# lmjakt/kmer_hasheR

Hardware: NVIDIA B200
Metric: kmers_indexed_per_s (higher is better)
Workload: dtype u64

## Files before the change

### kmer_hasher_b200/csrc/api.cu

```cuda
#include <cstdarg>
#include <cstdio>
#include <cstring>
#include <ctime>
#include <algorithm>
#include <atomic>
#include <condition_variable>
#include <deque>
#include <thread>
#include <map>
#include <mutex>
#include <string>
#include <type_traits>
#include <vector>

#include "../../include/kmergpu.h"
#include "common.cuh"
#include "csr.cuh"
#include "lookback.cuh"
#include "probe.cuh"
#include "sort.cuh"
#include "windows.cuh"

using namespace kmg;

static thread_local char g_err[512] = "";
static int fail(int code, const char *fmt, ...) {
  va_list ap;
  va_start(ap, fmt);
  vsnprintf(g_err, sizeof g_err, fmt, ap);
  va_end(ap);
  return code;
}
#define CU(call)                                                                                   \
  do {                                                                                             \
    cudaError_t e_ = (call);                                                                       \
    if (e_ != cudaSuccess) {                                                                       \
      int code_ = (e_ == cudaErrorMemoryAllocation) ? KMG_ERR_NOMEM                                \
                  : (e_ == cudaErrorNoDevice || e_ == cudaErrorInsufficientDriver) ? KMG_ERR_NODEV \
                                                                                   : KMG_ERR_CUDA; \
      return fail(code_, "%s: %s (%s:%d)", #call, cudaGetErrorString(e_), __FILE__, __LINE__);     \
    }                                                                                              \
  } while (0)
#define TRY(call)            \
  do {                       \
    int rc_ = (call);        \
    if (rc_ != KMG_OK) return rc_; \
  } while (0)

extern "C" const char *kmg_last_error(void) { return g_err; }
extern "C" int kmg_version(void) { return 100; }

struct Ctx {
  int device = 0;
  bool ready = false;
  cudaStream_t own = nullptr, copy = nullptr;
  cudaStream_t user = nullptr;
  bool use_user = false;
  cudaEvent_t ev[8] = {nullptr, nullptr, nullptr, nullptr, nullptr, nullptr, nullptr, nullptr};
  int sms = 148;
  cudaStream_t stream() const { return use_user ? user : own; }
};
static thread_local Ctx g_ctx;

static int ctx_init() {
  Ctx &c = g_ctx;
  if (c.ready) {
    CU(cudaSetDevice(c.device));
    return KMG_OK;
  }
  int n = 0;
  cudaError_t e = cudaGetDeviceCount(&n);
  if (e != cudaSuccess || n == 0)
    return fail(KMG_ERR_NODEV, "no CUDA device: %s (libkmergpu has no CPU path)", cudaGetErrorString(e));
  if (c.device >= n) return fail(KMG_ERR_ARG, "device %d out of range (have %d)", c.device, n);
  CU(cudaSetDevice(c.device));
  cudaDeviceProp prop;
  CU(cudaGetDeviceProperties(&prop, c.device));
  if (prop.major != 10 || prop.minor != 0)
    return fail(KMG_ERR_NODEV, "device %d is sm_%d%d; libkmergpu is built for sm_100a (B200) only", c.device, prop.major, prop.minor);
  c.sms = prop.multiProcessorCount;
  CU(cudaStreamCreateWithFlags(&c.own, cudaStreamNonBlocking));
  CU(cudaStreamCreateWithFlags(&c.copy, cudaStreamNonBlocking));
  for (auto &ev : c.ev) CU(cudaEventCreateWithFlags(&ev, cudaEventDisableTiming));
  c.ready = true;
  return KMG_OK;
}

extern "C" int kmg_device_count(int *n) {
  if (!n) return fail(KMG_ERR_ARG, "n is NULL");
  cudaError_t e = cudaGetDeviceCount(n);
  if (e != cudaSuccess) { *n = 0; return fail(KMG_ERR_NODEV, "cudaGetDeviceCount: %s", cudaGetErrorString(e)); }
  return KMG_OK;
}
extern "C" int kmg_set_device(int device) {
  if (device < 0) return fail(KMG_ERR_ARG, "negative device");
  if (g_ctx.ready && g_ctx.device != device) {
    g_ctx = Ctx();
  }
  g_ctx.device = device;
  return ctx_init();
}
extern "C" int kmg_set_stream(void *s) {
  g_ctx.user = (cudaStream_t)s;
  g_ctx.use_user = true;
  return KMG_OK;
}
extern "C" int kmg_unset_stream(void) { g_ctx.use_user = false; return KMG_OK; }
extern "C" void *kmg_host_alloc(size_t bytes) {
  void *p = nullptr;
  if (ctx_init() != KMG_OK) return nullptr;
  if (cudaMallocHost(&p, bytes ? bytes : 1) != cudaSuccess) { fail(KMG_ERR_NOMEM, "cudaMallocHost(%zu) failed", bytes); return nullptr; }
  return p;
}
extern "C" void kmg_host_free(void *p) { if (p) cudaFreeHost(p); }

struct ProfEntry { double ms = 0; uint64_t launches = 0; double bytes = 0; };
struct ProfPending { std::string name; cudaEvent_t a, b; };
static std::mutex g_prof_mu;
static bool g_prof_on = false;
static std::map<std::string, ProfEntry> g_prof;
static std::vector<ProfPending> g_prof_pending;
static std::vector<cudaEvent_t> g_prof_free;
static uint64_t g_launches = 0;

static cudaEvent_t prof_event() {
  if (!g_prof_free.empty()) { cudaEvent_t e = g_prof_free.back(); g_prof_free.pop_back(); return e; }
  cudaEvent_t e;
  cudaEventCreate(&e);
  return e;
}
static void prof_resolve() {
  for (auto &p : g_prof_pending) {
    float ms = 0;
    if (cudaEventSynchronize(p.b) == cudaSuccess && cudaEventElapsedTime(&ms, p.a, p.b) == cudaSuccess) {
      g_prof[p.name].ms += ms;
    }
    g_prof_free.push_back(p.a);
    g_prof_free.push_back(p.b);
  }
  g_prof_pending.clear();
}
struct LaunchScope {
  const char *name;
  cudaStream_t s;
  cudaEvent_t a = nullptr, b = nullptr;
  bool on;
  LaunchScope(const char *n, cudaStream_t st) : name(n), s(st) {
    std::lock_guard<std::mutex> g(g_prof_mu);
    on = g_prof_on;
    ++g_launches;
    if (on) { a = prof_event(); b = prof_event(); cudaEventRecord(a, s); }
  }
  ~LaunchScope() {
    if (!on) return;
    cudaEventRecord(b, s);
    std::lock_guard<std::mutex> g(g_prof_mu);
    g_prof[name].launches++;
    g_prof_pending.push_back({name, a, b});
  }
};
static void prof_bytes(const char *name, double bytes) {
  std::lock_guard<std::mutex> g(g_prof_mu);
  if (g_prof_on) g_prof[name].bytes += bytes;
}
#define LAUNCH(name, stream, ...)                                                              \
  do {                                                                                         \
    { LaunchScope ls_(name, stream); __VA_ARGS__; }                                            \
    cudaError_t le_ = cudaGetLastError();                                                      \
    if (le_ != cudaSuccess) return fail(KMG_ERR_CUDA, "launch %s: %s", name, cudaGetErrorString(le_)); \
  } while (0)

extern "C" int kmg_profile_enable(int on) { std::lock_guard<std::mutex> g(g_prof_mu); g_prof_on = on != 0; return KMG_OK; }
extern "C" int kmg_profile_reset(void) {
  std::lock_guard<std::mutex> g(g_prof_mu);
  prof_resolve();
  g_prof.clear();
  return KMG_OK;
}
extern "C" int kmg_profile_count(void) {
  std::lock_guard<std::mutex> g(g_prof_mu);
  prof_resolve();
  return (int)g_prof.size();
}
extern "C" int kmg_profile_get(int i, const char **name, double *total_ms, uint64_t *launches, double *algo_bytes) {
  std::lock_guard<std::mutex> g(g_prof_mu);
  prof_resolve();
  if (i < 0 || i >= (int)g_prof.size()) return fail(KMG_ERR_ARG, "profile index out of range");
  auto it = g_prof.begin();
  std::advance(it, i);
  if (name) *name = it->first.c_str();
  if (total_ms) *total_ms = it->second.ms;
  if (launches) *launches = it->second.launches;
  if (algo_bytes) *algo_bytes = it->second.bytes;
  return KMG_OK;
}
extern "C" uint64_t kmg_launch_count(void) { std::lock_guard<std::mutex> g(g_prof_mu); return g_launches; }

struct Arena {
  struct Block { void *p; size_t cap; cudaStream_t last; bool synced; };
  std::mutex mu;
  std::multimap<size_t, Block> cache;
  std::map<void *, Block> live;
  size_t cached_bytes = 0, limit = 0;

  static size_t round_up(size_t bytes) {
    if (bytes < (size_t(1) << 20)) return (bytes + 511) & ~size_t(511);
    return (bytes + (size_t(2) << 20) - 1) & ~((size_t(2) << 20) - 1);
  }
  void trim_locked() {
    for (auto &kv : cache) cudaFree(kv.second.p);
    cache.clear();
    cached_bytes = 0;
  }
  int get(void **out, size_t bytes, cudaStream_t s) {
    const size_t cap = round_up(bytes ? bytes : 1);
    std::unique_lock<std::mutex> g(mu);
    auto it = cache.lower_bound(cap);
    if (it != cache.end() && it->first <= cap + std::max(cap / 4, size_t(1) << 20)) {
      Block b = it->second;
      cache.erase(it);
      cached_bytes -= b.cap;
      g.unlock();
      if (!b.synced && b.last != s) cudaStreamSynchronize(b.last);
      g.lock();
      b.last = s; b.synced = false;
      live[b.p] = b;
      *out = b.p;
      return KMG_OK;
    }
    void *p = nullptr;
    cudaError_t e = cudaMalloc(&p, cap);
    if (e != cudaSuccess) {
      cudaGetLastError();
      trim_locked();
      e = cudaMalloc(&p, cap);
    }
    if (e != cudaSuccess) { cudaGetLastError(); return fail(KMG_ERR_NOMEM, "device allocation of %zu bytes failed: %s", cap, cudaGetErrorString(e)); }
    live[p] = Block{p, cap, s, false};
    *out = p;
    return KMG_OK;
  }
  void put(void *p, cudaStream_t s, bool synced) {
    if (!p) return;
    std::lock_guard<std::mutex> g(mu);
    auto it = live.find(p);
    if (it == live.end()) {
      for (auto &kv : cache) if (kv.second.p == p) return;
      cudaFree(p);
      return;
    }
    Block b = it->second;
    live.erase(it);
    b.last = s; b.synced = synced;
    if (limit == 0) {
      const char *e = getenv("KMERGPU_CACHE_MB");
      size_t fr = 0, tot = 0;
      if (e && atoll(e) >= 0) limit = (size_t)atoll(e) << 20;
      else limit = cudaMemGetInfo(&fr, &tot) == cudaSuccess ? tot / 4 : (size_t(32) << 30);
      if (limit == 0) limit = 1;
    }
    if (cached_bytes + b.cap > limit) trim_locked();
    cache.emplace(b.cap, b);
    cached_bytes += b.cap;
  }
};
static Arena g_arena[64];

static void stage_release();
extern "C" int kmg_trim(void) {
  TRY(ctx_init());
  cudaStreamSynchronize(g_ctx.stream());
  Arena &a = g_arena[g_ctx.device & 63];
  std::lock_guard<std::mutex> g(a.mu);
  for (auto &kv : a.cache) if (!kv.second.synced && kv.second.last && kv.second.last != g_ctx.stream()) cudaStreamSynchronize(kv.second.last);
  a.trim_locked();
  stage_release();
  return KMG_OK;
}
extern "C" uint64_t kmg_cached_bytes(void) {
  Arena &a = g_arena[g_ctx.device & 63];
  std::lock_guard<std::mutex> g(a.mu);
  return a.cached_bytes;
}

template <typename T>
static int dalloc(T **p, size_t count, cudaStream_t s) {
  *p = nullptr;
  return g_arena[g_ctx.device & 63].get((void **)p, (count ? count : 1) * sizeof(T), s);
}
template <typename T>
static void dfree(T *&p, cudaStream_t s) {
  if (p) g_arena[g_ctx.device & 63].put((void *)p, s, false);
  p = nullptr;
}

extern "C" void kmg_host_copy(void *dst, const void *src, size_t n);
class CopyPool {
  struct Task { char *dst; const char *src; size_t n; int group; };
  std::mutex mu;
  std::condition_variable cv_work, cv_done;
  std::deque<Task> q;
  int pending[8] = {0, 0, 0, 0, 0, 0, 0, 0};
  std::vector<std::thread> th;
  bool stop = false;
  void run() {
    for (;;) {
      Task t;
      {
        std::unique_lock<std::mutex> l(mu);
        cv_work.wait(l, [&] { return stop || !q.empty(); });
        if (q.empty()) return;
        t = q.front();
        q.pop_front();
      }
      kmg_host_copy(t.dst, t.src, t.n);
      {
        std::lock_guard<std::mutex> l(mu);
        if (--pending[t.group & 7] == 0) cv_done.notify_all();
      }
    }
  }
 public:
  int threads() {
    std::lock_guard<std::mutex> l(mu);
    if (th.empty()) {
      const char *e = getenv("KMERGPU_COPY_THREADS");
      int n = e ? atoi(e) : (int)std::thread::hardware_concurrency() / 2;
      n = std::max(1, std::min(n, 8));
      for (int i = 0; i < n; ++i) th.emplace_back([this] { run(); });
    }
    return (int)th.size();
  }
  void submit(int group, void *dst, const void *src, size_t n) {
    const int parts = threads();
    const size_t piece = ((n + parts - 1) / parts + 4095) & ~size_t(4095);
    std::lock_guard<std::mutex> l(mu);
    for (size_t off = 0; off < n; off += piece) {
      q.push_back(Task{(char *)dst + off, (const char *)src + off, std::min(piece, n - off), group});
      ++pending[group & 7];
    }
    cv_work.notify_all();
  }
  void wait(int group) {
    std::unique_lock<std::mutex> l(mu);
    cv_done.wait(l, [&] { return pending[group & 7] == 0; });
  }
  ~CopyPool() {
    { std::lock_guard<std::mutex> l(mu); stop = true; }
    cv_work.notify_all();
    for (auto &t : th) t.join();
  }
};
static CopyPool g_pool;
constexpr size_t STAGE_BYTES = size_t(64) << 20;
constexpr int STAGE_SLOTS = 3;
struct Staging {
  std::mutex mu;
  char *slot[STAGE_SLOTS] = {nullptr, nullptr, nullptr};
  int ensure() {
    for (auto &p : slot)
      if (!p && cudaMallocHost((void **)&p, STAGE_BYTES) != cudaSuccess) { cudaGetLastError(); return fail(KMG_ERR_NOMEM, "pinned staging allocation failed"); }
    return KMG_OK;
  }
  void release() { for (auto &p : slot) { if (p) cudaFreeHost(p); p = nullptr; } }
};
static Staging g_stage;
static void stage_release() { std::lock_guard<std::mutex> gs(g_stage.mu); g_stage.release(); }
static bool staged_transfers() {
  static int on = -1;
  if (on < 0) { const char *e = getenv("KMERGPU_STAGING"); on = !(e && e[0] == '0'); }
  return on == 1;
}

static int staged_upload(void *d_dst, const void *h_src, size_t bytes, cudaStream_t s) {
  std::lock_guard<std::mutex> g(g_stage.mu);
  TRY(g_stage.ensure());
  cudaEvent_t *ev = g_ctx.ev + 4;
  int c = 0;
  for (size_t off = 0; off < bytes; off += STAGE_BYTES, ++c) {
    const int sl = c % STAGE_SLOTS;
    const size_t n = std::min(STAGE_BYTES, bytes - off);
    if (c >= STAGE_SLOTS) CU(cudaEventSynchronize(ev[sl]));
    g_pool.submit(c, g_stage.slot[sl], (const char *)h_src + off, n);
    g_pool.wait(c);
    CU(cudaMemcpyAsync((char *)d_dst + off, g_stage.slot[sl], n, cudaMemcpyHostToDevice, s));
    CU(cudaEventRecord(ev[sl], s));
  }
  CU(cudaStreamSynchronize(s));
  return KMG_OK;
}

enum PtrKind { PK_HOST_PAGEABLE, PK_HOST_PINNED, PK_DEVICE };
static PtrKind ptr_kind(const void *p) {
  cudaPointerAttributes a;
  if (cudaPointerGetAttributes(&a, p) != cudaSuccess) { cudaGetLastError(); return PK_HOST_PAGEABLE; }
  if (a.type == cudaMemoryTypeDevice || a.type == cudaMemoryTypeManaged) return PK_DEVICE;
  if (a.type == cudaMemoryTypeHost) return PK_HOST_PINNED;
  return PK_HOST_PAGEABLE;
}

struct DevSeq {
  uint8_t *buf = nullptr;
  uint8_t *base = nullptr;
  int64_t len = 0;
};
static int upload_seq(const void *src, int64_t len, cudaStream_t s, DevSeq *out) {
  size_t cap = 16 + (size_t)((len + 15) / 16) * 16 + 16;
  TRY(dalloc(&out->buf, cap, s));
  out->base = out->buf + 16;
  out->len = len;
  CU(cudaMemsetAsync(out->buf, 0, 16, s));
  CU(cudaMemsetAsync(out->buf + cap - 32, 0, 32, s));
  if (len > (int64_t)(8 << 20) && staged_transfers() && ptr_kind(src) == PK_HOST_PAGEABLE) return staged_upload(out->base, src, (size_t)len, s);
  if (len > 0) CU(cudaMemcpyAsync(out->base, src, (size_t)len, cudaMemcpyDefault, s));
  return KMG_OK;
}

struct kmg_index {
  int device = 0;
  int k = 0;
  uint64_t U = 0, N = 0;
  uint64_t P = 0, multi = 0;
  uint32_t maxc = 0;
  bool have_stats = false;
  bool grouped = false;
  int hbits = 0;
  bool unstable = false;
  uint64_t *ukeys = nullptr;
  uint32_t *ustart = nullptr;
  uint32_t *pos = nullptr;
  std::mutex mu;
  uint4 *hash = nullptr;
  uint64_t hash_nb = 0;
  int hash_hbits = 0;
  uint32_t *multi_u = nullptr;
  uint64_t *pair_off = nullptr;
};
struct kmg_query {
  const kmg_index *idx = nullptr;
  uint64_t H = 0, M = 0;
  int32_t *hit_i = nullptr;
  uint32_t *hit_start = nullptr;
  uint64_t *row_off = nullptr;
};

constexpr int HIST_THREADS = 512, HIST_ITEMS = 16, HIST_TILE = HIST_THREADS * HIST_ITEMS;
constexpr int RLE_THREADS = 256, RLE_ITEMS = 16, RLE_TILE = RLE_THREADS * RLE_ITEMS;
constexpr int PROBE_THREADS = 256, PROBE_ITEMS = 8, PROBE_TILE = PROBE_THREADS * PROBE_ITEMS;
constexpr int COMPACT_ITEMS = 8, COMPACT_TILE = PROBE_THREADS * COMPACT_ITEMS;
constexpr int EMIT_THREADS = 256, EMIT_TILE = EMIT_THREADS * 8;
constexpr int PIDX_THREADS = 256, PIDX_ITEMS = 8, PIDX_TILE = PIDX_THREADS * PIDX_ITEMS;

static int g_sort_shape = -1;
static int g_rank_override = -1;
static std::atomic<int> g_rank_dev[64];
static std::atomic<uint64_t> g_unstable_rebuilds{0};
static std::atomic<uint64_t> g_region_rebuilds{0};
static uint32_t g_sort_dbg = 0;
static int lane_order_failures(uint32_t *failures);
static bool log_on();

static int rank_variant() {
  if (g_rank_override >= 0) return g_rank_override;
  const int dev = g_ctx.device & 63;
  int v = g_rank_dev[dev].load(std::memory_order_acquire);
  if (v == 0) {
    const char *e = getenv("KMG_SORT_RANK");
    if (e) v = atoi(e) == 3 ? 2 : 1;
    else {
      uint32_t f = 1;
      v = (lane_order_failures(&f) == KMG_OK && f == 0) ? 2 : 1;
      if (log_on()) fprintf(stderr, "[kmergpu] device %d lane-order self-test: %u failures -> rank variant %d\n", dev, f, v == 2 ? 3 : 0);
    }
    int expect = 0;
    g_rank_dev[dev].compare_exchange_strong(expect, v, std::memory_order_acq_rel);
    v = g_rank_dev[dev].load(std::memory_order_acquire);
  }
  return v == 2 ? 3 : 0;
}
static void demote_rank_variant() {
  g_rank_dev[g_ctx.device & 63].store(1, std::memory_order_release);
  g_unstable_rebuilds.fetch_add(1);
  if (g_rank_override >= 3) g_rank_override = -1;
  if (log_on()) fprintf(stderr, "[kmergpu] device %d: position lists not ascending after a one-atomic sort pass; switching to the bitmap variant\n", g_ctx.device);
}

struct SortPlan { int rb, passes; int bits() const { return rb * passes; } };
static int g_hash_bits = 0;
static int g_hash_rb = 0;
static int g_no_regions = 0;
static int g_scatter_shape = 0;
static int g_scatter_bitmap = 0;
static int g_hash_cas = 0;
static int g_fix_cap = 0;
static SortPlan grouped_plan(int64_t n_upper) {
  if (g_hash_bits > 0) {
    const int rb = g_hash_rb > 0 && g_hash_bits % g_hash_rb == 0 ? g_hash_rb : (g_hash_bits % 8 == 0 ? 8 : 9);
    return SortPlan{rb, g_hash_bits / rb};
  }
  if (g_hash_rb > 0) return SortPlan{g_hash_rb, (36 + g_hash_rb - 1) / g_hash_rb};
  return n_upper <= (int64_t)400000000 ? SortPlan{8, 4} : SortPlan{8, 5};
}
static bool grouped_for(int k, int order, int64_t ) {
  return order == KMG_ORDER_GROUPED && 2 * k > 40;
}

static unsigned long long *g_trace = nullptr;
static int g_trace_tiles = 0;
extern "C" int kmg_trace_read(unsigned long long *host, int tiles) {
  if (!g_trace || tiles > g_trace_tiles) return -1;
  return cudaMemcpy(host, g_trace, (size_t)tiles * 64, cudaMemcpyDeviceToHost) == cudaSuccess ? 0 : -4;
}
extern "C" int kmg_tune(const char *key, int value) {
  if (key && !strcmp(key, "sort_cfg")) {
    if (value != -1 && value != 0 && value != 3 && value != 4) return fail(KMG_ERR_ARG, "sort_cfg must be -1 (auto), 0 (bitmap), 3 (one atomic) or 4 (tests: unstable on purpose)");
    g_rank_override = value;
    return KMG_OK;
  }
  if (key && !strcmp(key, "sort_shape")) {
    if (value < -1 || value > 2) return fail(KMG_ERR_ARG, "sort_shape out of range");
    g_sort_shape = value;
    return KMG_OK;
  }
  if (key && !strcmp(key, "sort_dbg")) { g_sort_dbg = (uint32_t)value; return KMG_OK; }
  if (key && !strcmp(key, "fix_cap")) { g_fix_cap = value > 0 ? value : 0; return KMG_OK; }
  if (key && !strcmp(key, "hash_cas")) { g_hash_cas = value != 0; return KMG_OK; }
  if (key && !strcmp(key, "scatter_bitmap")) { g_scatter_bitmap = value != 0; return KMG_OK; }
  if (key && !strcmp(key, "scatter_shape")) { g_scatter_shape = value; return KMG_OK; }
  if (key && !strcmp(key, "no_regions")) { g_no_regions = value; return KMG_OK; }
  if (key && !strcmp(key, "hash_bits")) {
    if (value != 0 && (value < 8 || value > 56 || (value % 8 && value % 9 && value % 10))) return fail(KMG_ERR_ARG, "hash_bits must be 0 (auto) or a multiple of 8, 9 or 10 in [8,56]");
    g_hash_bits = value;
    return KMG_OK;
  }
  if (key && !strcmp(key, "hash_rb")) {
    if (value != 0 && (value < 8 || value > 10)) return fail(KMG_ERR_ARG, "hash_rb must be 0, 8, 9 or 10");
    g_hash_rb = value;
    return KMG_OK;
  }
  if (key && !strcmp(key, "reset_rank")) {
    for (auto &v : g_rank_dev) v.store(0);
    return KMG_OK;
  }
  if (key && !strcmp(key, "sort_trace")) {
    if (g_trace) { cudaFree(g_trace); g_trace = nullptr; }
    g_trace_tiles = value;
    if (value > 0) { if (cudaMalloc(&g_trace, (size_t)value * 64) != cudaSuccess) return fail(KMG_ERR_NOMEM, "trace alloc"); cudaMemset(g_trace, 0, (size_t)value * 64); }
    return KMG_OK;
  }
  return fail(KMG_ERR_ARG, "unknown tuning key");
}
extern "C" int64_t kmg_tune_get(const char *key, int64_t arg) {
  if (key && !strcmp(key, "rank_variant")) return ctx_init() == KMG_OK ? rank_variant() : -1;
  if (key && !strcmp(key, "unstable_rebuilds")) return (int64_t)g_unstable_rebuilds.load();
  if (key && !strcmp(key, "region_rebuilds")) return (int64_t)g_region_rebuilds.load();
  if (key && !strcmp(key, "hash_bits")) return grouped_plan(arg).bits();
  if (key && !strcmp(key, "hash_rb")) return grouped_plan(arg).rb;
  return -1;
}
static int lane_order_failures(uint32_t *failures) {
  TRY(ctx_init());
  cudaStream_t s = g_ctx.stream();
  uint32_t *bad = nullptr;
  TRY(dalloc(&bad, 1, s));
  CU(cudaMemsetAsync(bad, 0, 4, s));
  LAUNCH("lane_order_selftest", s, lane_order_selftest_kernel<<<g_ctx.sms * 4, 256, 0, s>>>(bad));
  CU(cudaMemcpyAsync(failures, bad, 4, cudaMemcpyDeviceToHost, s));
  CU(cudaStreamSynchronize(s));
  dfree(bad, s);
  return KMG_OK;
}
extern "C" int kmg_selftest_lane_order(uint32_t *failures) {
  if (!failures) return fail(KMG_ERR_ARG, "failures is NULL");
  return lane_order_failures(failures);
}
static_assert(2 * (sizeof(PassSmem<PassCfg<256, 28, 2, 3, 4, 8>, false>) + 1024) <= 196 * 1024, "the record pass's tile outgrew the 196 KB carve-out");
constexpr int REGION_SAMPLE_STRIDE = 251;
constexpr int SORT_TILE_MIN = 4096;

template <class Cfg, bool FROM_SEQ, class BinFn, class NextFn, bool HAS_NEXT, bool PEER = false, bool SEGS = false>
static int launch_pass_cfg(const char *name, const PassParams<BinFn, NextFn> &P, int64_t n_upper, cudaStream_t s, int extra_tiles = 0) {
  using S = PassSmem<Cfg, FROM_SEQ>;
  if constexpr (!FROM_SEQ && !PEER && !SEGS) {
    if (P.segs) return launch_pass_cfg<Cfg, FROM_SEQ, BinFn, NextFn, HAS_NEXT, PEER, true>(name, P, n_upper, s, extra_tiles);
  }
  auto kern = scatter_pass_kernel<Cfg, FROM_SEQ, BinFn, NextFn, HAS_NEXT, PEER, SEGS>;
  CU(cudaFuncSetAttribute(kern, cudaFuncAttributeMaxDynamicSharedMemorySize, (int)sizeof(S)));
  const int64_t tiles = ceil_div<int64_t>(n_upper, Cfg::TILE) + extra_tiles;
  if (tiles == 0) return KMG_OK;
  LAUNCH(name, s, kern<<<(unsigned)tiles, Cfg::THREADS, sizeof(S), s>>>(P));
  return KMG_OK;
}
template <bool FROM_SEQ, class BinFn, class NextFn, bool HAS_NEXT>
static int launch_pass(const char *name, const PassParams<BinFn, NextFn> &P, int64_t n_upper, cudaStream_t s, int rb = RADIX_BITS, int extra_tiles = 0) {
  const int rank = rank_variant();
  const int shape = g_sort_shape < 0 ? (rb == 8 ? 1 : 0)
                                     : (rb == 8) ? ((FROM_SEQ && g_sort_shape == 0) ? 1 : g_sort_shape) : (g_sort_shape == 2 ? 0 : g_sort_shape);
#define KMG_GO(T, I, M, RK, RB) return launch_pass_cfg<PassCfg<T, I, M, RK, (RK >= 3 ? 4 : 8), RB>, FROM_SEQ, BinFn, NextFn, HAS_NEXT>(name, P, n_upper, s, extra_tiles)
#define KMG_SHAPES(RK, RB)                         \
  do {                                             \
    if (shape == 1) KMG_GO(256, 28, 2, RK, RB);    \
    KMG_GO(256, 24, 2, RK, RB);                    \
  } while (0)
  if (rb == 8) {
    if (rank == 4) KMG_GO(256, 24, 2, 4, 8);
    if (shape == 2) { if (rank == 3) KMG_GO(256, 20, 3, 3, 8); else KMG_GO(256, 20, 3, 0, 8); }
    if (rank == 3) KMG_SHAPES(3, 8); else KMG_SHAPES(0, 8);
  } else if (rb == 9) {
    if (rank == 4) KMG_GO(256, 24, 2, 4, 9);
    if (rank == 3) KMG_SHAPES(3, 9); else KMG_SHAPES(0, 9);
  } else if (rb == 10) {
    if (rank == 3) KMG_GO(256, 24, 2, 3, 10); else KMG_GO(256, 24, 2, 0, 10);
  }
#undef KMG_SHAPES
#undef KMG_GO
  return fail(KMG_ERR_ARG, "bad sort configuration");
}

static uint32_t record_tile(int rb) {
  const int shape = g_sort_shape < 0 ? (rb == 8 ? 1 : 0) : (rb == 8) ? g_sort_shape : (g_sort_shape == 2 ? 0 : g_sort_shape);
  if (rank_variant() == 4 || rb == 10) return 256 * 24;
  return shape == 1 ? 256 * 28 : shape == 2 ? 256 * 20 : 256 * 24;
}

struct SortScratch {
  uint32_t *small = nullptr;
  uint64_t *status = nullptr;
  size_t small_words = 0, status_words = 0;
  static constexpr size_t H = (size_t)(MAX_PASSES + 1) * MAX_NB;
  uint32_t *hist(int r) const { return small + (size_t)r * MAX_NB; }
  uint32_t *gbase(int r) const { return small + H + (size_t)r * MAX_NB; }
  uint32_t *common() const { return small + 2 * H; }
  uint32_t *ticket(int i) const { return small + 2 * H + RADIX + i; }
  IndexStats *stats() const { return reinterpret_cast<IndexStats *>(small + 2 * H + RADIX + 16); }
};
static int scratch_clear(SortScratch &sc, cudaStream_t s) {
  CU(cudaMemsetAsync(sc.small, 0, sc.small_words * 4, s));
  CU(cudaMemsetAsync(sc.status, 0, sc.status_words * sizeof(uint64_t), s));
  return KMG_OK;
}
static int scratch_alloc(SortScratch &sc, int64_t n_upper, cudaStream_t s, int rb = RADIX_BITS) {
  sc.small_words = 2 * SortScratch::H + RADIX + 16 + sizeof(IndexStats) / 4;
  TRY(dalloc(&sc.small, sc.small_words, s));
  const size_t tiles = (size_t)ceil_div<int64_t>(n_upper > 0 ? n_upper : 1, SORT_TILE_MIN) + MAX_SEGS + 1;
  sc.status_words = tiles << rb;
  TRY(dalloc(&sc.status, sc.status_words, s));
  return scratch_clear(sc, s);
}
static void scratch_free(SortScratch &sc, cudaStream_t s) { dfree(sc.small, s); dfree(sc.status, s); }

template <class... A>
static int launch_scan_hist(int rb, cudaStream_t s, A... args) {
  if (rb == 8) LAUNCH("scan_hist", s, scan_hist_kernel<256><<<1, 256, 0, s>>>(args...));
  else if (rb == 9) LAUNCH("scan_hist", s, scan_hist_kernel<512><<<1, 512, 0, s>>>(args...));
  else if (rb == 10) LAUNCH("scan_hist", s, scan_hist_kernel<1024><<<1, 1024, 0, s>>>(args...));
  else return fail(KMG_ERR_ARG, "bad digit width");
  return KMG_OK;
}

static int finish_index(kmg_index *ix, SortScratch &sc, uint64_t *keys_sorted, uint32_t *pos_sorted,
                        int64_t n_upper, cudaStream_t s, bool hashed = false) {
  IndexStats *st = sc.stats();
  uint64_t *ukeys = nullptr;
  uint32_t *ustart = nullptr;
  Pair64 *status2 = nullptr;
  const int64_t tiles = ceil_div<int64_t>(n_upper > 0 ? n_upper : 1, RLE_TILE);
  TRY(dalloc(&ukeys, (size_t)n_upper, s));
  TRY(dalloc(&ustart, (size_t)n_upper + 1, s));
  TRY(dalloc(&status2, (size_t)tiles, s));
  CU(cudaMemsetAsync(status2, 0, (size_t)tiles * sizeof(Pair64), s));
  LAUNCH("rle", s, rle_kernel<RLE_THREADS, RLE_ITEMS><<<(unsigned)tiles, RLE_THREADS, 0, s>>>(
                       keys_sorted, pos_sorted, st, ukeys, ustart, status2, sc.ticket(MAX_PASSES + 1), hashed));
  IndexStats h;
  CU(cudaMemcpyAsync(&h, st, sizeof h, cudaMemcpyDeviceToHost, s));
  CU(cudaStreamSynchronize(s));
  ix->N = h.n; ix->U = h.U; ix->unstable = h.unstable != 0;
  ix->have_stats = false;
  dfree(status2, s);
  if (h.U * 2 < (uint64_t)n_upper) {
    uint64_t *uk2; uint32_t *us2;
    TRY(dalloc(&uk2, (size_t)h.U, s));
    TRY(dalloc(&us2, (size_t)h.U + 1, s));
    CU(cudaMemcpyAsync(uk2, ukeys, h.U * sizeof(uint64_t), cudaMemcpyDeviceToDevice, s));
    CU(cudaMemcpyAsync(us2, ustart, (h.U + 1) * sizeof(uint32_t), cudaMemcpyDeviceToDevice, s));
    dfree(ukeys, s); dfree(ustart, s);
    ukeys = uk2; ustart = us2;
  }
  ix->ukeys = ukeys; ix->ustart = ustart; ix->pos = pos_sorted;
  const double N = (double)h.n, U = (double)h.U;
  prof_bytes("rle", 12 * N + 12 * U);
  return KMG_OK;
}

static int sort_tail(SortScratch &sc, SortPlan plan, int first_pass, bool has_next, uint64_t *&ka, uint32_t *&pa, uint64_t *&kb,
                     uint32_t *&pb, int64_t n_upper, cudaStream_t s, uint32_t *final_pos = nullptr, const TileSegs *seg0 = nullptr, int nsegs0 = 0,
                     int end_pass = -1) {
  const int R = plan.passes, rb = plan.rb;
  const uint32_t mask = (1u << rb) - 1;
  for (int r = first_pass; r < (end_pass > 0 ? end_pass : R); ++r) {
    PassParams<DigitBin, DigitBin> P{};
    P.keys_in = ka; P.pos_in = pa; P.keys_out = kb; P.pos_out = (final_pos && r == R - 1) ? final_pos : pb;
    P.gbase = sc.gbase(r); P.hist_next = sc.hist(r + 1);
    P.status = sc.status; P.ticket = sc.ticket(r); P.epoch = (uint32_t)(r + 1);
    P.n_records = &sc.stats()->n;
    P.segs = r == first_pass ? seg0 : nullptr;
    const int extra = r == first_pass && seg0 ? nsegs0 : 0;
    P.bin = DigitBin{r * rb, mask}; P.next = DigitBin{(r + 1) * rb, mask};
    P.dbg = g_sort_dbg;
    P.trace = (r == 2 && g_trace && ceil_div<int64_t>(n_upper, SORT_TILE_MIN) <= g_trace_tiles) ? g_trace : nullptr;
    if (has_next && r + 1 < R) {
      TRY((launch_pass<false, DigitBin, DigitBin, true>("sort_pass_hist", P, n_upper, s, rb, extra)));
      TRY(launch_scan_hist(rb, s, sc.hist(r + 1), sc.gbase(r + 1), (uint64_t *)nullptr));
    } else {
      TRY((launch_pass<false, DigitBin, DigitBin, false>("sort_pass", P, n_upper, s, rb, extra)));
    }
    std::swap(ka, kb);
    std::swap(pa, pb);
  }
  return KMG_OK;
}

static int fix_groups(SortScratch &sc, int bits, uint64_t *keys, uint32_t *pos, uint64_t *sk, uint32_t *sp, int64_t n_upper, cudaStream_t s,
                      uint32_t *h_cnt , uint32_t **fixmem_out) {
  FixLists fl{};
  uint32_t *fixmem = nullptr;
  fl.small_cap = g_fix_cap > 0 ? (uint32_t)g_fix_cap : (uint32_t)std::max<int64_t>(1 << 20, n_upper / 8);
  fl.big_cap = 1 << 16;
  const size_t words = 4 + CLAIM_SLOTS + 2 * (size_t)fl.small_cap + 2 * (size_t)fl.big_cap;
  TRY(dalloc(&fixmem, words, s));
  *fixmem_out = fixmem;
  CU(cudaMemsetAsync(fixmem, 0, (4 + CLAIM_SLOTS) * sizeof(uint32_t), s));
  fl.counters = fixmem; fl.claim = fixmem + 4;
  fl.small_tasks = reinterpret_cast<uint2 *>(fixmem + 4 + CLAIM_SLOTS);
  fl.big_tasks = fl.small_tasks + fl.small_cap;
  const unsigned dgrid = (unsigned)std::min<int64_t>(ceil_div<int64_t>(n_upper, 256 * 8), (int64_t)g_ctx.sms * 16);
  if (bits == 32) LAUNCH("group_detect", s, group_detect_kernel<true><<<dgrid, 256, 0, s>>>(keys, sc.stats(), bits, fl));
  else LAUNCH("group_detect", s, group_detect_kernel<false><<<dgrid, 256, 0, s>>>(keys, sc.stats(), bits, fl));
  LAUNCH("small_fix", s, small_fix_kernel<<<g_ctx.sms * 4, 128, 0, s>>>(keys, pos, fl));
  LAUNCH("big_fix", s, big_fix_kernel<1024><<<g_ctx.sms, 1024, 0, s>>>(keys, pos, sk, sp, fl));
  CU(cudaMemcpyAsync(h_cnt, fl.counters, 4 * sizeof(uint32_t), cudaMemcpyDeviceToHost, s));
  return KMG_OK;
}

static int build_grouped(const SeqView &sv, SortPlan plan, kmg_index *ix, SortScratch &sc, uint64_t *&ka, uint32_t *&pa, uint64_t *&kb,
                         uint32_t *&pb, int64_t n_upper, cudaStream_t s, bool *overflow, bool regions, bool *region_overflow) {
  const int R = plan.passes, rb = plan.rb, NB = 1 << rb;
  const uint32_t mask = (1u << rb) - 1;
  uint64_t *kr = nullptr, *d_counts = nullptr;
  uint32_t *pr = nullptr, *d_over = nullptr;
  TileSegs *segs = nullptr;
  uint32_t h_over = 0;
  regions = regions && R > 1 && NB <= MAX_SEGS && n_upper <= (int64_t)1600000000;
  const uint32_t cap = (uint32_t)(((uint64_t)(n_upper / NB) * 5 / 4 + 4096 + 15) & ~uint64_t(15));
  if (regions && g_no_regions == 2) {
  } else if (regions && n_upper >= (int64_t)REGION_SAMPLE_STRIDE * 4096) {
    uint32_t *d_s = nullptr, h_est = 0;
    TRY(dalloc(&d_s, (size_t)MAX_NB + 1, s));
    int rc0 = KMG_OK;
    if (cudaMemsetAsync(d_s, 0, (MAX_NB + 1) * sizeof(uint32_t), s) != cudaSuccess) rc0 = fail(KMG_ERR_CUDA, "memset failed");
    if (rc0 == KMG_OK) {
      const unsigned g = (unsigned)std::min<int64_t>(ceil_div<int64_t>(n_upper / REGION_SAMPLE_STRIDE, 256), (int64_t)g_ctx.sms * 8);
      region_sample_kernel<<<g, 256, 0, s>>>(sv, REGION_SAMPLE_STRIDE, mask, d_s);
      region_estimate_kernel<<<1, 256, 0, s>>>(d_s, NB, REGION_SAMPLE_STRIDE, d_s + MAX_NB);
      if (cudaMemcpyAsync(&h_est, d_s + MAX_NB, 4, cudaMemcpyDeviceToHost, s) != cudaSuccess || cudaStreamSynchronize(s) != cudaSuccess)
        rc0 = fail(KMG_ERR_CUDA, "region estimate failed: %s", cudaGetErrorString(cudaGetLastError()));
    }
    dfree(d_s, s);
    TRY(rc0);
    if ((uint64_t)h_est * 10 > (uint64_t)cap * 9) regions = false;
  } else if (regions) {
    regions = false;
  }
  auto body = [&]() -> int {
    PassParams<DigitBin, DigitBin> P{};
    P.sv = sv; P.keys_out = ka; P.pos_out = pa;
    P.gbase = sc.gbase(0); P.hist_next = sc.hist(1);
    P.status = sc.status; P.ticket = sc.ticket(0); P.epoch = 1;
    P.hashed = 1;
    P.dbg = g_sort_dbg;
    P.bin = DigitBin{0, mask}; P.next = DigitBin{rb, mask};
    if (regions) {
      TRY(dalloc(&kr, (size_t)NB * cap, s));
      TRY(dalloc(&pr, (size_t)NB * cap, s));
      TRY(dalloc(&d_counts, (size_t)MAX_SEGS, s));
      TRY(dalloc(&d_over, 4, s));
      TRY(dalloc(&segs, 1, s));
      CU(cudaMemsetAsync(d_counts, 0, MAX_SEGS * sizeof(uint64_t), s));
      LAUNCH("region_gbase", s, region_gbase_kernel<<<1, 256, 0, s>>>(sc.gbase(0), NB, cap, d_over));
      P.keys_out = kr; P.pos_out = pr;
      P.bin_counts = d_counts; P.bin_cap = cap; P.bin_overflow = d_over;
      TRY((launch_pass<true, DigitBin, DigitBin, true>("sort_pass_seq", P, n_upper, s, rb)));
      TRY(launch_scan_hist(rb, s, sc.hist(1), sc.gbase(1), (uint64_t *)nullptr));
      LAUNCH("tile_segs", s, tile_segs_kernel<<<1, MAX_SEGS, 0, s>>>(d_counts, NB, (uint64_t)cap, record_tile(rb), segs, &sc.stats()->n));
      CU(cudaMemcpyAsync(&h_over, d_over, 4, cudaMemcpyDeviceToHost, s));
      TRY(sort_tail(sc, plan, 1, true, kr, pr, ka, pa, n_upper, s, nullptr, segs, NB, 2));
      std::swap(kr, ka); std::swap(pr, pa);
      TRY(sort_tail(sc, plan, 2, true, ka, pa, kb, pb, n_upper, s));
    } else {
      const int64_t tiles = ceil_div<int64_t>(n_upper, HIST_TILE);
      const unsigned hgrid = (unsigned)std::min<int64_t>(tiles, (int64_t)g_ctx.sms * 2);
      LAUNCH("hist_seq", s, hist_seq_kernel<HIST_THREADS, HIST_ITEMS, HashDigitBin><<<hgrid, HIST_THREADS, 0, s>>>(sv, sc.hist(0), HashDigitBin{0, mask}));
      TRY(launch_scan_hist(rb, s, sc.hist(0), sc.gbase(0), &sc.stats()->n));
      if (R > 1) {
        TRY((launch_pass<true, DigitBin, DigitBin, true>("sort_pass_seq", P, n_upper, s, rb)));
        TRY(launch_scan_hist(rb, s, sc.hist(1), sc.gbase(1), (uint64_t *)nullptr));
      } else {
        TRY((launch_pass<true, DigitBin, DigitBin, false>("sort_pass_seq", P, n_upper, s, rb)));
      }
      TRY(sort_tail(sc, plan, 1, true, ka, pa, kb, pb, n_upper, s));
    }
    return KMG_OK;
  };
  int rc = body();
  uint32_t h_cnt[4] = {0, 0, 0, 0};
  uint32_t *fixmem = nullptr;
  if (rc == KMG_OK) rc = fix_groups(sc, plan.bits(), ka, pa, kb, pb, n_upper, s, h_cnt, &fixmem);
  if (rc == KMG_OK) rc = finish_index(ix, sc, ka, pa, n_upper, s, true);
  dfree(fixmem, s);
  dfree(kr, s); dfree(pr, s); dfree(d_counts, s); dfree(d_over, s); dfree(segs, s);
  *overflow = h_cnt[2] != 0;
  *region_overflow = h_over != 0;
  if (log_on()) fprintf(stderr, "[kmergpu] grouped build on %d bits: %u short and %u long groups fixed\n", plan.bits(), h_cnt[0], h_cnt[1]);
  ix->hbits = plan.bits();
  const double N = (double)ix->N, L = (double)sv.avail;
  if (!regions) prof_bytes("hist_seq", L);
  prof_bytes("sort_pass_seq", L + 12 * N);
  if (R > 2) prof_bytes("sort_pass_hist", 24 * N * (R - 2));
  if (R > 1) prof_bytes("sort_pass", 24 * N);
  prof_bytes("group_detect", 8 * N);
  return rc;
}

static int build_attempt(const SeqView &sv, int k, kmg_index *ix, int order, cudaStream_t s) {
  const int64_t n_upper = sv.nstarts;
  SortScratch sc;
  uint64_t *ka = nullptr, *kb = nullptr;
  uint32_t *pa = nullptr, *pb = nullptr;
  auto body = [&]() -> int {
    const int R = num_passes(k);
    const bool grouped = grouped_for(k, order, n_upper);
    const SortPlan gp = grouped_plan(n_upper);
    TRY(scratch_alloc(sc, n_upper, s, grouped ? gp.rb : RADIX_BITS));
    TRY(dalloc(&ka, (size_t)n_upper, s));
    TRY(dalloc(&pa, (size_t)n_upper, s));
    if (R > 1) { TRY(dalloc(&kb, (size_t)n_upper, s)); TRY(dalloc(&pb, (size_t)n_upper, s)); }
    if (grouped) {
      bool overflow = false, region_overflow = false;
      TRY(build_grouped(sv, gp, ix, sc, ka, pa, kb, pb, n_upper, s, &overflow, g_no_regions != 1, &region_overflow));
      if (region_overflow) {
        g_region_rebuilds.fetch_add(1);
        if (log_on()) fprintf(stderr, "[kmergpu] a first-pass bin outgrew its region: rebuilding with the histogram sweep\n");
        void *old[3] = {ix->ukeys, ix->ustart, nullptr};
        for (void *p : old) g_arena[ix->device & 63].put(p, s, false);
        ix->ukeys = nullptr; ix->ustart = nullptr; ix->pos = nullptr; ix->hbits = 0; ix->unstable = false;
        TRY(scratch_clear(sc, s));
        overflow = false;
        TRY(build_grouped(sv, gp, ix, sc, ka, pa, kb, pb, n_upper, s, &overflow, false, &region_overflow));
      }
      if (!overflow) { pa = nullptr; ix->grouped = true; return KMG_OK; }
      void *old[3] = {ix->ukeys, ix->ustart, nullptr};
      for (void *p : old) g_arena[ix->device & 63].put(p, s, false);
      ix->ukeys = nullptr; ix->ustart = nullptr; ix->pos = nullptr; ix->hbits = 0;
      scratch_free(sc, s);
      TRY(scratch_alloc(sc, n_upper, s, RADIX_BITS));
    }
    const int64_t tiles = ceil_div<int64_t>(n_upper, HIST_TILE);
    const unsigned hgrid = (unsigned)std::min<int64_t>(tiles, (int64_t)g_ctx.sms * 2);
    LAUNCH("hist_all", s, hist_all_kernel<HIST_THREADS, HIST_ITEMS><<<hgrid, HIST_THREADS, 0, s>>>(sv, sc.common(), sc.hist(0), MAX_NB));
    LAUNCH("hist_finish", s, hist_finish_kernel<<<R, RADIX, 0, s>>>(k, sc.common(), sc.hist(0), sc.gbase(0), MAX_NB, &sc.stats()->n));
    {
      PassParams<DigitBin, DigitBin> P{};
      P.sv = sv; P.keys_out = ka; P.pos_out = pa;
      P.gbase = sc.gbase(0);
      P.status = sc.status; P.ticket = sc.ticket(0); P.epoch = 1;
      P.dbg = g_sort_dbg;
      P.bin = DigitBin{0}; P.next = DigitBin{RADIX_BITS};
      TRY((launch_pass<true, DigitBin, DigitBin, false>("sort_pass_seq", P, n_upper, s)));
    }
    TRY(sort_tail(sc, SortPlan{RADIX_BITS, R}, 1, false, ka, pa, kb, pb, n_upper, s));
    TRY(finish_index(ix, sc, ka, pa, n_upper, s));
    pa = nullptr;
    const double N = (double)ix->N, L = (double)sv.avail;
    prof_bytes("hist_all", L);
    prof_bytes("sort_pass_seq", L + 12 * N);
    if (R > 1) prof_bytes("sort_pass", 24 * N * (R - 1));
    return KMG_OK;
  };
  const int rc = body();
  dfree(ka, s); dfree(kb, s); dfree(pa, s); dfree(pb, s);
  scratch_free(sc, s);
  return rc;
}

static void release_index_arrays(kmg_index *ix, cudaStream_t s) {
  void *ptrs[3] = {ix->ukeys, ix->ustart, ix->pos};
  for (void *p : ptrs) g_arena[ix->device & 63].put(p, s, false);
  ix->ukeys = nullptr; ix->ustart = nullptr; ix->pos = nullptr;
  ix->grouped = false; ix->hbits = 0; ix->unstable = false;
}

static int build_from_view(const SeqView &sv, int k, kmg_index **out, int order = KMG_ORDER_SORTED) {
  cudaStream_t s = g_ctx.stream();
  kmg_index *ix = new (std::nothrow) kmg_index();
  if (!ix) return fail(KMG_ERR_NOMEM, "host allocation failed");
  ix->device = g_ctx.device;
  ix->k = k;
  const int64_t n_upper = sv.nstarts;
  if (n_upper <= 0) {
    int rc = dalloc(&ix->ustart, 1, s);
    if (rc == KMG_OK && cudaMemsetAsync(ix->ustart, 0, 4, s) != cudaSuccess) rc = fail(KMG_ERR_CUDA, "memset failed");
    if (rc != KMG_OK) { delete ix; return rc; }
    cudaStreamSynchronize(s);
    *out = ix;
    return KMG_OK;
  }
  if (n_upper > (int64_t)INT32_MAX) { delete ix; return fail(KMG_ERR_RANGE, "%lld windows exceed the 32-bit coordinates of the reference", (long long)n_upper); }
  int rc = build_attempt(sv, k, ix, order, s);
  if (rc == KMG_OK && ix->unstable) {
    const bool was_atomic = rank_variant() >= 3;
    release_index_arrays(ix, s);
    if (!was_atomic) rc = fail(KMG_ERR_CUDA, "internal error: position lists not ascending after a stable sort");
    else {
      demote_rank_variant();
      rc = build_attempt(sv, k, ix, order, s);
      if (rc == KMG_OK && ix->unstable) rc = fail(KMG_ERR_CUDA, "internal error: position lists not ascending after a stable sort");
    }
  }
  if (rc != KMG_OK) { cudaStreamSynchronize(s); kmg_free(ix); return rc; }
  *out = ix;
  return KMG_OK;
}

static double wall_ms() {
  timespec ts;
  clock_gettime(CLOCK_MONOTONIC, &ts);
  return ts.tv_sec * 1e3 + ts.tv_nsec * 1e-6;
}
static bool log_on() {
  static int on = -1;
  if (on < 0) { const char *e = getenv("KMERGPU_LOG"); on = e && e[0] == '1'; }
  return on == 1;
}

extern "C" int kmg_build(const char *seq, int64_t len, int k, kmg_index **out) {
  return kmg_build_ordered(seq, len, k, KMG_ORDER_GROUPED, out);
}
extern "C" int kmg_index_order(const kmg_index *ix) { return !ix ? fail(KMG_ERR_ARG, "index is NULL") : (ix->grouped ? KMG_ORDER_GROUPED : KMG_ORDER_SORTED); }

extern "C" int kmg_build_ordered(const char *seq, int64_t len, int k, int order, kmg_index **out) {
  if (!out) return fail(KMG_ERR_ARG, "out is NULL");
  if (order != KMG_ORDER_SORTED && order != KMG_ORDER_GROUPED) return fail(KMG_ERR_ARG, "order must be KMG_ORDER_SORTED or KMG_ORDER_GROUPED");
  *out = nullptr;
  if (k < 1 || k > KMG_MAX_K) return fail(KMG_ERR_K, "k must be a positive integer less than 1+MAX_K");
  if (len < 0 || (len > 0 && !seq)) return fail(KMG_ERR_ARG, "bad sequence pointer/length");
  const double t0 = wall_ms();
  TRY(ctx_init());
  cudaStream_t s = g_ctx.stream();
  DevSeq ds;
  TRY(upload_seq(seq, len, s, &ds));
  const double t1 = wall_ms();
  SeqView sv;
  sv.base = ds.base; sv.nstarts = len - k + 1 > 0 ? len - k + 1 : 0; sv.avail = len; sv.s0 = 0; sv.L = len; sv.k = k;
  int rc = build_from_view(sv, k, out, order);
  dfree(ds.buf, s);
  if (log_on())
    fprintf(stderr, "[kmergpu] build len=%lld k=%d: upload(enqueue) %.3f ms, build %.3f ms (host wall clock)\n", (long long)len, k, t1 - t0, wall_ms() - t1);
  return rc;
}

extern "C" int kmg_free(kmg_index *ix) {
  if (!ix) return KMG_OK;
  int prev = -1;
  cudaGetDevice(&prev);
  cudaSetDevice(ix->device);
  const bool mine = g_ctx.ready && g_ctx.device == ix->device;
  if (mine) cudaStreamSynchronize(g_ctx.stream()); else cudaDeviceSynchronize();
  void *ptrs[6] = {ix->ukeys, ix->ustart, ix->pos, ix->hash, ix->multi_u, ix->pair_off};
  for (void *p : ptrs) g_arena[ix->device & 63].put(p, nullptr, true);
  cudaGetLastError();
  if (prev >= 0) cudaSetDevice(prev);
  delete ix;
  return KMG_OK;
}

static int use_index(const kmg_index *ix);
static int ensure_stats(const kmg_index *cix) {
  kmg_index *ix = const_cast<kmg_index *>(cix);
  std::lock_guard<std::mutex> g(ix->mu);
  if (ix->have_stats) return KMG_OK;
  if (ix->U == 0) { ix->P = 0; ix->multi = 0; ix->maxc = 0; ix->have_stats = true; return KMG_OK; }
  TRY(use_index(ix));
  cudaStream_t s = g_ctx.stream();
  IndexStats *st = nullptr, h;
  TRY(dalloc(&st, 1, s));
  auto body = [&]() -> int {
    CU(cudaMemsetAsync(st, 0, sizeof(IndexStats), s));
    const unsigned sgrid = (unsigned)std::min<uint64_t>(ceil_div<uint64_t>(ix->U, 256 * 16), (uint64_t)g_ctx.sms * 8);
    LAUNCH("stats", s, stats_kernel<256><<<sgrid, 256, 0, s>>>(ix->ustart, ix->U, st));
    CU(cudaMemcpyAsync(&h, st, sizeof h, cudaMemcpyDeviceToHost, s));
    CU(cudaStreamSynchronize(s));
    return KMG_OK;
  };
  const int rc = body();
  dfree(st, s);
  TRY(rc);
  ix->P = h.P; ix->multi = h.multi; ix->maxc = h.maxc;
  ix->have_stats = true;
  prof_bytes("stats", 4.0 * (double)ix->U);
  return KMG_OK;
}

extern "C" int kmg_sizes(const kmg_index *ix, uint64_t *U, uint64_t *N, uint64_t *P) {
  if (!ix) return fail(KMG_ERR_ARG, "index is NULL");
  if (P) { TRY(ensure_stats(ix)); *P = ix->P; }
  if (U) *U = ix->U;
  if (N) *N = ix->N;
  return KMG_OK;
}
extern "C" int kmg_index_k(const kmg_index *ix) { return ix ? ix->k : fail(KMG_ERR_ARG, "index is NULL"); }
extern "C" int kmg_index_stats(const kmg_index *ix, uint64_t *multi, uint32_t *max_count) {
  if (!ix) return fail(KMG_ERR_ARG, "index is NULL");
  TRY(ensure_stats(ix));
  if (multi) *multi = ix->multi;
  if (max_count) *max_count = ix->maxc;
  return KMG_OK;
}

static int use_index(const kmg_index *ix) {
  if (!ix) return fail(KMG_ERR_ARG, "index is NULL");
  TRY(ctx_init());
  if (ix->device != g_ctx.device)
    return fail(KMG_ERR_ARG, "the index lives on device %d but this thread works on device %d: call kmg_set_device(%d) first", ix->device, g_ctx.device, ix->device);
  return KMG_OK;
}

template <class Emit>
static int stream_rows_staged(uint64_t total, size_t row_bytes, void *out, Emit emit) {
  std::lock_guard<std::mutex> g(g_stage.mu);
  TRY(g_stage.ensure());
  cudaStream_t s = g_ctx.stream(), cs = g_ctx.copy;
  const uint64_t chunk_rows = std::max<uint64_t>(1, STAGE_BYTES / row_bytes);
  const int64_t nchunks = (int64_t)ceil_div<uint64_t>(total, chunk_rows);
  uint64_t *blk = nullptr;
  char *buf[2] = {nullptr, nullptr};
  TRY(dalloc(&blk, (size_t)ceil_div<uint64_t>(chunk_rows, EMIT_TILE), s));
  int rc = dalloc(&buf[0], chunk_rows * row_bytes, s);
  if (rc == KMG_OK && nchunks > 1) rc = dalloc(&buf[1], chunk_rows * row_bytes, s);
  cudaEvent_t *ev = g_ctx.ev;
  int64_t issued = 0, retired = 0;
  while (rc == KMG_OK && retired < nchunks) {
    while (rc == KMG_OK && issued < nchunks && issued - retired < 2) {
      const int64_t c = issued;
      const int b = (int)(c & 1), sl = (int)(c % STAGE_SLOTS);
      const uint64_t first = (uint64_t)c * chunk_rows, rows = std::min<uint64_t>(chunk_rows, total - first);
      if (c >= STAGE_SLOTS) g_pool.wait((int)(c - STAGE_SLOTS));
      if (c >= 2) cudaStreamWaitEvent(s, ev[4 + (int)((c - 2) % STAGE_SLOTS)], 0);
      rc = emit(first, rows, (void *)buf[b], blk, s);
      if (rc != KMG_OK) break;
      cudaEventRecord(ev[b], s);
      cudaStreamWaitEvent(cs, ev[b], 0);
      if (cudaMemcpyAsync(g_stage.slot[sl], buf[b], rows * row_bytes, cudaMemcpyDeviceToHost, cs) != cudaSuccess)
        rc = fail(KMG_ERR_CUDA, "device->host copy failed: %s", cudaGetErrorString(cudaGetLastError()));
      cudaEventRecord(ev[4 + sl], cs);
      ++issued;
    }
    if (rc != KMG_OK) break;
    const int64_t c = retired;
    const int sl = (int)(c % STAGE_SLOTS);
    const uint64_t first = (uint64_t)c * chunk_rows, rows = std::min<uint64_t>(chunk_rows, total - first);
    if (cudaEventSynchronize(ev[4 + sl]) != cudaSuccess) { rc = fail(KMG_ERR_CUDA, "device->host copy failed: %s", cudaGetErrorString(cudaGetLastError())); break; }
    g_pool.submit((int)c, (char *)out + first * row_bytes, g_stage.slot[sl], rows * row_bytes);
    ++retired;
  }
  for (int64_t c = std::max<int64_t>(0, retired - STAGE_SLOTS); c < retired; ++c) g_pool.wait((int)c);
  cudaStreamSynchronize(cs);
  cudaStreamSynchronize(s);
  dfree(buf[0], s); dfree(buf[1], s); dfree(blk, s);
  if (rc == KMG_OK) {
    cudaError_t e = cudaGetLastError();
    if (e != cudaSuccess) rc = fail(KMG_ERR_CUDA, "extraction failed: %s", cudaGetErrorString(e));
  }
  return rc;
}

template <class Emit>
static int stream_rows(uint64_t total, size_t row_bytes, void *out, uint64_t chunk_rows, Emit emit) {
  if (total == 0) return KMG_OK;
  cudaStream_t s = g_ctx.stream();
  const bool to_device = ptr_kind(out) == PK_DEVICE;
  if (!to_device) chunk_rows = std::min<uint64_t>(chunk_rows, total);
  uint64_t *blk = nullptr;
  TRY(dalloc(&blk, (size_t)ceil_div<uint64_t>(to_device ? total : chunk_rows, EMIT_TILE), s));
  if (to_device) {
    int rc = emit((uint64_t)0, total, out, blk, s);
    if (rc == KMG_OK && cudaStreamSynchronize(s) != cudaSuccess) rc = fail(KMG_ERR_CUDA, "extraction failed: %s", cudaGetErrorString(cudaGetLastError()));
    dfree(blk, s);
    return rc;
  }
  if (staged_transfers() && total * row_bytes > (uint64_t)(8 << 20) && ptr_kind(out) == PK_HOST_PAGEABLE) {
    dfree(blk, s);
    return stream_rows_staged(total, row_bytes, out, emit);
  }
  char *buf[2] = {nullptr, nullptr};
  int rc = dalloc(&buf[0], chunk_rows * row_bytes, s);
  if (rc == KMG_OK && total > chunk_rows) rc = dalloc(&buf[1], chunk_rows * row_bytes, s);
  if (rc != KMG_OK) { dfree(buf[0], s); dfree(blk, s); return rc; }
  cudaStream_t cs = g_ctx.copy;
  cudaEvent_t *ev = g_ctx.ev;
  uint64_t done = 0;
  for (int c = 0; done < total && rc == KMG_OK; ++c, done += chunk_rows) {
    const int b = c & 1;
    const uint64_t rows = std::min<uint64_t>(chunk_rows, total - done);
    if (c >= 2) cudaStreamWaitEvent(s, ev[2 + b], 0);
    rc = emit(done, rows, (void *)buf[b], blk, s);
    if (rc != KMG_OK) break;
    cudaEventRecord(ev[b], s);
    cudaStreamWaitEvent(cs, ev[b], 0);
    if (cudaMemcpyAsync((char *)out + done * row_bytes, buf[b], rows * row_bytes, cudaMemcpyDeviceToHost, cs) != cudaSuccess)
      rc = fail(KMG_ERR_CUDA, "device->host copy failed: %s", cudaGetErrorString(cudaGetLastError()));
    cudaEventRecord(ev[2 + b], cs);
  }
  cudaStreamSynchronize(cs);
  cudaStreamSynchronize(s);
  dfree(buf[0], s); dfree(buf[1], s); dfree(blk, s);
  if (rc == KMG_OK) {
    cudaError_t e = cudaGetLastError();
    if (e != cudaSuccess) rc = fail(KMG_ERR_CUDA, "extraction failed: %s", cudaGetErrorString(e));
  }
  return rc;
// ... 1492 lines not shown
```

### kmer_hasher_b200/csrc/sort.cuh

```cuda
#pragma once
#include "common.cuh"
#include "lookback.cuh"
#include "windows.cuh"

namespace kmg {

struct DigitBin {
  static constexpr bool CHEAP = true;
  int shift;
  uint32_t mask = RADIX - 1;
  __device__ __forceinline__ uint32_t operator()(uint64_t key) const { return (uint32_t)(key >> shift) & mask; }
};
struct OwnerBin {
  static constexpr bool CHEAP = false;
  const uint64_t *spl;
  int nparts;
  __device__ __forceinline__ uint32_t operator()(uint64_t key) const {
    int lo = 0, hi = nparts - 1;
    while (lo < hi) {
      int mid = (lo + hi) >> 1;
      if (__ldg(spl + mid) <= key) lo = mid + 1; else hi = mid;
    }
    return (uint32_t)lo;
  }
};
struct HashOwnerBin {
  static constexpr bool CHEAP = false;
  OwnerBin ob;
  __device__ __forceinline__ uint32_t operator()(uint64_t key) const { return ob(mix64(key)); }
};
struct HashDigitBin {
  static constexpr bool CHEAP = true;
  int shift;
  uint32_t mask = RADIX - 1;
  __device__ __forceinline__ uint32_t operator()(uint64_t key) const { return (uint32_t)(mix64(key) >> shift) & mask; }
};
struct RangeBin {
  static constexpr bool CHEAP = true;
  uint32_t nparts;
  __device__ __forceinline__ uint32_t operator()(uint64_t h) const { return (uint32_t)__umul64hi(h, (uint64_t)nparts); }
};
struct NoBin {
  static constexpr bool CHEAP = true;
  __device__ __forceinline__ uint32_t operator()(uint64_t) const { return 0; }
};

constexpr int MAX_PEERS = 16;
struct PeerTable {
  uint64_t *keys[MAX_PEERS];
  uint32_t *pos[MAX_PEERS];
  int64_t delta[MAX_PEERS];
  uint64_t cap;
  uint64_t *counts[MAX_PEERS];
  uint32_t rank, region;
};
constexpr int MAX_SEGS = 512;
struct TileSegs {
  uint32_t tile_prefix[MAX_SEGS + 1];
  uint32_t count[MAX_SEGS];
  uint64_t stride, total;
  uint32_t nsegs, tile;
  uint32_t overflow, pad;
};
template <class BinFn, class NextFn>
struct PassParams {
  SeqView sv;
  const uint64_t *keys_in;
  const uint32_t *pos_in;
  uint64_t *keys_out;
  uint32_t *pos_out;
  const uint32_t *gbase;
  uint32_t *hist_next;
  uint64_t *status;
  uint32_t *ticket;
  const uint64_t *n_records;
  uint32_t epoch;
  uint32_t hashed;
  uint32_t pos_add;
  const PeerTable *peer;
  const TileSegs *segs;
  uint64_t *bin_counts;
  uint32_t bin_cap;
  uint32_t *bin_overflow;
  unsigned long long *trace;
  uint32_t dbg;
  BinFn bin;
  NextFn next;
};

template <int THREADS_, int ITEMS_, int MINBLOCKS_, int RANK_ = 3, int LB_ = 4, int RB_ = RADIX_BITS>
struct PassCfg {
  static constexpr int THREADS = THREADS_, ITEMS = ITEMS_, MINBLOCKS = MINBLOCKS_, RANK = RANK_, LB = LB_, RB = RB_;
  static constexpr int TILE = THREADS * ITEMS;
  static constexpr int NB = 1 << RB_;
  static constexpr int BPT = NB >= THREADS_ ? NB / THREADS_ : 1;
  static_assert(RANK_ == 0 || RANK_ == 3 || RANK_ == 4, "rank variants: 0 bitmap, 3 one atomic, 4 = 3 made unstable on purpose (tests)");
  static_assert(NB < THREADS_ || NB % THREADS_ == 0, "bins per thread");
  static_assert(BPT == 1 || BPT == 2 || BPT == 4, "a thread's bins are moved as one vector");
};

template <class Cfg, bool FROM_SEQ>
struct PassSmem {
  static constexpr int TILE = Cfg::TILE;
  static constexpr int WARPS = Cfg::THREADS / 32;
  static constexpr int NB = Cfg::NB;
  using PosT = typename std::conditional<FROM_SEQ, uint16_t, uint32_t>::type;
  uint64_t keys[TILE];
  PosT pos[TILE];
  alignas(16) uint32_t whist[WARPS][NB];
  uint32_t match[Cfg::RANK == 0 ? WARPS * NB : 1];
  int32_t goff[NB];
  uint32_t next[NB];
  uint32_t scratch[32];
  uint32_t tile;
  uint32_t seg_tp[MAX_SEGS + 1];
  uint32_t skip_write;
  alignas(8) uint64_t bar[WARPS];
  alignas(8) uint64_t bar2[WARPS];
  uint32_t bstart[MAX_PEERS], bcnt[MAX_PEERS];
  PeerTable peer;
  TileCodes<FROM_SEQ ? TILE : 16> tc;
};

__global__ void lane_order_selftest_kernel(uint32_t *bad) {
  constexpr int STEPS = 8;
  __shared__ uint32_t tab[8][RADIX];
  __shared__ uint32_t sim[8][RADIX];
  __shared__ uint8_t dig[8][STEPS][32];
  __shared__ uint32_t got[8][STEPS][32];
  const unsigned lane = threadIdx.x & 31u, warp = threadIdx.x >> 5;
  uint32_t fails = 0;
  for (int rep = 0; rep < 32; ++rep) {
    for (int pattern = 0; pattern < 6; ++pattern) {
      for (int b = lane; b < RADIX; b += 32) { tab[warp][b] = 0; sim[warp][b] = 0; }
      __syncwarp();
      uint32_t d[STEPS], g[STEPS];
#pragma unroll
      for (int j = 0; j < STEPS; ++j) {
        switch (pattern) {
          case 0: d[j] = 7; break;
          case 1: d[j] = (lane + j) & 1; break;
          case 2: d[j] = (lane >> 3) + (j & 1); break;
          case 3: d[j] = ((lane + 7 * j) * 2654435761u + rep * 40503u) >> 29; break;
          case 4: d[j] = ((lane + 32 * j) * 2246822519u + rep * 97u) & 255u; break;
          default: d[j] = (lane % 3 == 0) ? 200 : ((lane * 5 + j) & 255u); break;
        }
      }
#pragma unroll
      for (int j = 0; j < STEPS; ++j) g[j] = atomicAdd(&tab[warp][d[j]], 1u);
#pragma unroll
      for (int j = 0; j < STEPS; ++j) { dig[warp][j][lane] = (uint8_t)d[j]; got[warp][j][lane] = g[j]; }
      __syncwarp();
      if (lane == 0) {
        for (int j = 0; j < STEPS; ++j)
          for (int l = 0; l < 32; ++l)
            if (got[warp][j][l] != sim[warp][dig[warp][j][l]]++) ++fails;
      }
      __syncwarp();
    }
  }
  if (fails) atomicAdd(bad, fails);
}

template <int BPT> struct WordVec;
template <> struct WordVec<1> { using T = uint32_t; };
template <> struct WordVec<2> { using T = uint2; };
template <> struct WordVec<4> { using T = uint4; };
template <int BPT>
__device__ __forceinline__ void load_words(const uint32_t *p, uint32_t (&v)[BPT]) {
  const typename WordVec<BPT>::T t = *reinterpret_cast<const typename WordVec<BPT>::T *>(p);
  if constexpr (BPT == 1) v[0] = t;
  else if constexpr (BPT == 2) { v[0] = t.x; v[1] = t.y; }
  else { v[0] = t.x; v[1] = t.y; v[2] = t.z; v[3] = t.w; }
}
template <int BPT>
__device__ __forceinline__ void store_words(uint32_t *p, const uint32_t (&v)[BPT]) {
  typename WordVec<BPT>::T t;
  if constexpr (BPT == 1) t = v[0];
  else if constexpr (BPT == 2) { t.x = v[0]; t.y = v[1]; }
  else { t.x = v[0]; t.y = v[1]; t.z = v[2]; t.w = v[3]; }
  *reinterpret_cast<typename WordVec<BPT>::T *>(p) = t;
}
template <int BPT>
__device__ __forceinline__ void ld_status(const uint64_t *p, uint64_t (&w)[BPT]) {
  if constexpr (BPT == 1) w[0] = ld_relaxed_u64(p);
  else {
#pragma unroll
    for (int q = 0; q < BPT; q += 2)
      asm volatile("ld.relaxed.gpu.global.v2.u64 {%0,%1}, [%2];" : "=l"(w[q]), "=l"(w[q + 1]) : "l"(p + q) : "memory");
  }
}
template <int BPT>
__device__ __forceinline__ void st_status(uint64_t *p, const uint64_t (&w)[BPT]) {
  if constexpr (BPT == 1) st_relaxed_u64(p, w[0]);
  else {
#pragma unroll
    for (int q = 0; q < BPT; q += 2)
      asm volatile("st.relaxed.gpu.global.v2.u64 [%0], {%1,%2};" ::"l"(p + q), "l"(w[q]), "l"(w[q + 1]) : "memory");
  }
}

__device__ __forceinline__ uint32_t smem_addr(const void *p) { return (uint32_t)__cvta_generic_to_shared(p); }
__device__ __forceinline__ void bulk_load_arm(uint64_t *bar, void *dst, const void *src, uint32_t bytes) {
  const uint32_t b = smem_addr(bar), d = smem_addr(dst);
  asm volatile("mbarrier.init.shared::cta.b64 [%0], 1;" ::"r"(b) : "memory");
  asm volatile("fence.proxy.async.shared::cta;" ::: "memory");
  asm volatile("mbarrier.arrive.expect_tx.shared::cta.b64 _, [%0], %1;" ::"r"(b), "r"(bytes) : "memory");
  asm volatile("cp.async.bulk.shared::cluster.global.mbarrier::complete_tx::bytes [%0], [%1], %2, [%3];"
               ::"r"(d), "l"(src), "r"(bytes), "r"(b) : "memory");
}
__device__ __forceinline__ void bulk_load_wait(uint64_t *bar) {
  const uint32_t b = smem_addr(bar);
  asm volatile(
      "{\n\t.reg .pred p;\n\t"
      "KMG_WAIT:\n\t"
      "mbarrier.try_wait.parity.shared::cta.b64 p, [%0], 0;\n\t"
      "@p bra KMG_DONE;\n\t"
      "bra KMG_WAIT;\n\t"
      "KMG_DONE:\n\t}" ::"r"(b) : "memory");
}

template <class Cfg, bool FROM_SEQ, bool FULL, class BinFn, class NextFn, bool HAS_NEXT, bool PEER>
__device__ __forceinline__ void pass_tile(const PassParams<BinFn, NextFn> &P, PassSmem<Cfg, FROM_SEQ> &sm,
                                          const uint32_t tile, const int64_t q0, const int64_t n_in,
                                          const uint32_t (&gbase)[Cfg::BPT], const bool special) {
  using S = PassSmem<Cfg, FROM_SEQ>;
  constexpr int TILE = Cfg::TILE, THREADS = Cfg::THREADS, ITEMS = Cfg::ITEMS, WARPS = S::WARPS, NB = Cfg::NB, BPT = Cfg::BPT;
  const unsigned tid = threadIdx.x, lane = tid & 31u, warp = tid >> 5;
  const int t0 = warp * (32 * ITEMS) + lane;
  const bool owns = NB >= THREADS || tid < NB;
  const int b0 = tid * BPT;
#define KMG_STAMP(slot) do { if (P.trace && tid == 0) P.trace[(size_t)tile * 8 + (slot)] = clock64(); } while (0)
  KMG_STAMP(1);

  uint64_t key[ITEMS];
  uint32_t valid = FULL ? 0xFFFFFFFFu : 0u;
  bool bulk_pos = false;
  if constexpr (FROM_SEQ) {
#pragma unroll
    for (int i = 0; i < ITEMS; ++i) {
      const int t = t0 + i * 32;
      key[i] = tile_key<TILE>(sm.tc, t, P.sv.k);
      if (P.hashed) key[i] = mix64(key[i]);
      if constexpr (!FULL)
        if (tile_valid<TILE>(P.sv, sm.tc, q0, t, special)) valid |= 1u << i;
    }
  } else {
    const uint64_t *ksrc = P.keys_in + q0 + t0;
    bool bulk = false;
    if constexpr (FULL && !PEER) bulk = !(P.dbg & 8u) && (((uintptr_t)(P.keys_in + q0) & 15u) == 0);
    if constexpr (FULL && !PEER) bulk_pos = bulk && !(P.dbg & 16u) && (((uintptr_t)(P.pos_in + q0) & 15u) == 0);
    if (bulk) {
      if constexpr (FULL && !PEER) {
        uint64_t *stage = sm.keys + warp * (32 * ITEMS);
        if (lane == 0) {
          bulk_load_arm(&sm.bar[warp], stage, P.keys_in + q0 + warp * (32 * ITEMS), 32 * ITEMS * 8);
          if constexpr (!FROM_SEQ)
            if (bulk_pos) bulk_load_arm(&sm.bar2[warp], sm.pos + warp * (32 * ITEMS), P.pos_in + q0 + warp * (32 * ITEMS), 32 * ITEMS * 4);
        }
        __syncwarp();
        bulk_load_wait(&sm.bar[warp]);
#pragma unroll
        for (int i = 0; i < ITEMS; ++i) key[i] = stage[i * 32 + lane];
      }
    } else
#pragma unroll
    for (int i = 0; i < ITEMS; ++i) {
      if constexpr (FULL) key[i] = ld_stream_u64(ksrc + i * 32);
      else {
        key[i] = 0;
        const int64_t q = q0 + t0 + i * 32;
        if (q < n_in) { key[i] = ld_stream_u64(ksrc + i * 32); valid |= 1u << i; }
      }
    }
  }

  uint32_t rk[ITEMS];
  const unsigned lt = lanemask_lt();
  if (P.trace && tid == 0) { P.trace[(size_t)tile * 8 + 2] = (unsigned long long)(key[0] & 1) + clock64(); }
  uint32_t dpk[BinFn::CHEAP ? 1 : (ITEMS + 3) / 4] = {};
  if constexpr (!BinFn::CHEAP) {
#pragma unroll
    for (int i = 0; i < ITEMS; ++i) dpk[i >> 2] |= P.bin(key[i]) << (8 * (i & 3));
  }
#define KMG_BIN(i) (BinFn::CHEAP ? P.bin(key[i]) : ((dpk[(i) >> 2] >> (8 * ((i) & 3))) & 0xFFu))
  if constexpr (Cfg::RANK >= 3) {
#pragma unroll
    for (int ii = 0; ii < ITEMS; ++ii) {
      const int i = Cfg::RANK == 4 ? ITEMS - 1 - ii : ii;
      const uint32_t d = KMG_BIN(i);
      const bool ok = FULL || ((valid >> i) & 1u);
      uint32_t r = 0;
      if (ok) r = atomicAdd(&sm.whist[warp][d], 1u);
      rk[i] = (d << 16) | r;
      if constexpr (!FULL) __syncwarp();
    }
  } else {
    const uint32_t lanebit = 1u << lane;
    uint32_t *mrow = sm.match + warp * NB;
#pragma unroll
    for (int i = 0; i < ITEMS; ++i) {
      const uint32_t d = KMG_BIN(i);
      const bool ok = FULL || ((valid >> i) & 1u);
      __syncwarp();
      if (ok) atomicOr(&mrow[d], lanebit);
      __syncwarp();
      const uint32_t peers = ok ? mrow[d] : 0u;
      __syncwarp();
      uint32_t old = 0;
      if (ok && (peers & lt) == 0) {
        mrow[d] = 0;
        old = atomicAdd(&sm.whist[warp][d], (uint32_t)__popc(peers));
      }
      const uint32_t base = __shfl_sync(FULL_MASK_, old, (FULL || peers) ? (__ffs(peers) - 1) : 0);
      rk[i] = (d << 16) | (base + __popc(peers & lt));
    }
  }
#undef KMG_BIN
  KMG_STAMP(3);
  __syncthreads();
  KMG_STAMP(4);

  uint32_t cnt[BPT], lstart[BPT], tile_count;
  {
    uint32_t c[WARPS][BPT], mine = 0;
#pragma unroll
    for (int q = 0; q < BPT; ++q) cnt[q] = 0;
    if (owns) {
#pragma unroll
      for (int w = 0; w < WARPS; ++w) {
        load_words<BPT>(&sm.whist[w][b0], c[w]);
#pragma unroll
        for (int q = 0; q < BPT; ++q) cnt[q] += c[w][q];
      }
      uint64_t sw[BPT];
#pragma unroll
      for (int q = 0; q < BPT; ++q) { sw[q] = st_pack(tile == 0 ? ST_INCL : ST_AGG, P.epoch, cnt[q]); mine += cnt[q]; }
      st_status<BPT>(P.status + (size_t)tile * NB + b0, sw);
    }
    const uint32_t incl = warp_incl_scan(mine);
    if (lane == 31) sm.scratch[warp] = incl;
    __syncthreads();
    uint32_t add = 0, tot = 0;
#pragma unroll
    for (int j = 0; j < WARPS; ++j) {
      const uint32_t s = sm.scratch[j];
      if (j < (int)warp) add += s;
      tot += s;
    }
    tile_count = tot;
    uint32_t run = incl - mine + add;
#pragma unroll
    for (int q = 0; q < BPT; ++q) { lstart[q] = run; run += cnt[q]; }
    if (owns) {
      uint32_t r2[BPT];
#pragma unroll
      for (int q = 0; q < BPT; ++q) r2[q] = lstart[q];
#pragma unroll
      for (int w = 0; w < WARPS; ++w) {
        store_words<BPT>(&sm.whist[w][b0], r2);
#pragma unroll
        for (int q = 0; q < BPT; ++q) r2[q] += c[w][q];
      }
    }
  }
  __syncthreads();

#pragma unroll
  for (int i = 0; i < ITEMS; ++i)
    rk[i] = sm.whist[warp][rk[i] >> 16] + (rk[i] & 0xFFFFu);
#pragma unroll
  for (int i = 0; i < ITEMS; ++i)
    if (FULL || ((valid >> i) & 1u)) sm.keys[rk[i]] = key[i];
  if constexpr (FROM_SEQ) {
#pragma unroll
    for (int i = 0; i < ITEMS; ++i)
      if (FULL || ((valid >> i) & 1u)) sm.pos[rk[i]] = (uint16_t)(t0 + i * 32);
  } else {
    uint32_t val[ITEMS];
    if (bulk_pos) {
      bulk_load_wait(&sm.bar2[warp]);
#pragma unroll
      for (int i = 0; i < ITEMS; ++i) val[i] = sm.pos[t0 + i * 32];
      __syncthreads();
    } else
#pragma unroll
    for (int i = 0; i < ITEMS; ++i) {
      val[i] = (FULL || ((valid >> i) & 1u)) ? ld_stream_u32(P.pos_in + q0 + t0 + i * 32) : 0;
    }
#pragma unroll
    for (int i = 0; i < ITEMS; ++i)
      if (FULL || ((valid >> i) & 1u)) sm.pos[rk[i]] = val[i];
  }

  KMG_STAMP(5);
  if (owns) {
    uint64_t excl[BPT];
    bool done[BPT];
#pragma unroll
    for (int q = 0; q < BPT; ++q) { excl[q] = 0; done[q] = false; }
    if (tile > 0 && !(P.dbg & 1u)) {
      constexpr int LB = Cfg::LB;
      int64_t t = (int64_t)tile - 1;
      bool all_done = false;
      while (!all_done) {
        uint64_t w[LB][BPT];
#pragma unroll
        for (int j = 0; j < LB; ++j) {
          if (t - j >= 0) ld_status<BPT>(P.status + (size_t)(t - j) * NB + b0, w[j]);
          else {
#pragma unroll
            for (int q = 0; q < BPT; ++q) w[j][q] = st_pack(ST_INCL, P.epoch, 0);
          }
        }
        int adv = 0;
        bool stop = false;
#pragma unroll
        for (int j = 0; j < LB; ++j) {
          if (stop) break;
          bool ready = true;
#pragma unroll
          for (int q = 0; q < BPT; ++q) ready &= done[q] || st_flag(w[j][q], P.epoch) != 0;
          if (!ready) { stop = true; break; }
          bool pending = false;
#pragma unroll
          for (int q = 0; q < BPT; ++q) {
            if (!done[q]) {
              excl[q] += st_value(w[j][q]);
              if (st_flag(w[j][q], P.epoch) == ST_INCL) done[q] = true; else pending = true;
            }
          }
          ++adv;
          if (!pending) { all_done = true; stop = true; }
        }
        t -= adv;
        if (adv == 0) __nanosleep(40);
      }
      uint64_t sw[BPT];
#pragma unroll
      for (int q = 0; q < BPT; ++q) sw[q] = st_pack(ST_INCL, P.epoch, excl[q] + cnt[q]);
      st_status<BPT>(P.status + (size_t)tile * NB + b0, sw);
    }
#pragma unroll
    for (int q = 0; q < BPT; ++q) {
      const int64_t go = (int64_t)gbase[q] + (int64_t)excl[q] - (int64_t)lstart[q];
      sm.goff[b0 + q] = (int32_t)go;
      if constexpr (FROM_SEQ && !PEER) {
        if (P.bin_counts) {
          if (excl[q] + cnt[q] > P.bin_cap) { *P.bin_overflow = 1; sm.skip_write = 1; }
          if (q0 + TILE >= n_in) P.bin_counts[b0 + q] = excl[q] + cnt[q];
        }
      }
      if constexpr (PEER) {
        if (sm.peer.region && q0 + TILE >= n_in && b0 + q < MAX_PEERS && sm.peer.counts[b0 + q])
          sm.peer.counts[b0 + q][sm.peer.rank] = excl[q] + cnt[q];
        if (b0 + q < MAX_PEERS) { sm.bstart[b0 + q] = lstart[q]; sm.bcnt[b0 + q] = cnt[q]; }
      }
    }
  }
  __syncthreads();
  KMG_STAMP(6);

  bool drop = false;
  if constexpr (FROM_SEQ && !PEER) drop = sm.skip_write != 0;
  bool aligned_out = false;
  if constexpr (PEER) aligned_out = !(P.dbg & 4u);
  if (aligned_out) {
   if constexpr (PEER) {
    constexpr int OWNERS = NB < MAX_PEERS ? NB : MAX_PEERS;
    for (int b = 0; b < OWNERS; ++b) {
      const int cb = (int)sm.bcnt[b];
      if (cb == 0) continue;
      const int st = (int)sm.bstart[b];
      const int64_t go = sm.goff[b], delta = sm.peer.delta[b];
      uint64_t *kout = sm.peer.keys[b];
      uint32_t *pout = sm.peer.pos[b];
      const int mis = (int)((go + st + delta) & 31);
      for (int s = st - mis + (int)tid; s < st + cb; s += THREADS) {
        if (s < st) continue;
        const int64_t local = go + s, dst = local + delta;
        const bool room = (uint64_t)(sm.peer.region ? local : dst) < sm.peer.cap;
        const uint64_t kk = sm.keys[s];
        if (room && !(P.dbg & 2u)) {
          kout[dst] = kk;
          if constexpr (FROM_SEQ) pout[dst] = (uint32_t)(P.sv.s0 + q0 + 1) + P.pos_add + sm.pos[s];
          else pout[dst] = sm.pos[s];
        }
        if constexpr (HAS_NEXT) atomicAdd(&sm.next[P.next(kk)], 1u);
      }
    }
   }
  } else
#pragma unroll
  for (int j = 0; j < ITEMS; ++j) {
    const int s = j * THREADS + tid;
    if (FULL || s < (int)tile_count) {
      const uint64_t kk = sm.keys[s];
      const uint32_t b = P.bin(kk);
      int64_t dst = sm.goff[b] + s;
      uint64_t *kout = P.keys_out;
      uint32_t *pout = P.pos_out;
      bool room = true;
      if constexpr (PEER) {
        kout = sm.peer.keys[b]; pout = sm.peer.pos[b];
        const int64_t local = dst;
        dst += sm.peer.delta[b];
        room = (uint64_t)(sm.peer.region ? local : dst) < sm.peer.cap;
      }
      if constexpr (FROM_SEQ && !PEER) room = !drop;
      if (room && !(P.dbg & 2u)) {
        kout[dst] = kk;
        if constexpr (FROM_SEQ) pout[dst] = (uint32_t)(P.sv.s0 + q0 + 1) + P.pos_add + sm.pos[s];
        else pout[dst] = sm.pos[s];
      }
      if constexpr (HAS_NEXT) atomicAdd(&sm.next[P.next(kk)], 1u);
    }
  }
  KMG_STAMP(7);
#undef KMG_STAMP
}

template <class Cfg, bool FROM_SEQ, class BinFn, class NextFn, bool HAS_NEXT, bool PEER = false, bool SEGS = false>
__global__ void __launch_bounds__(Cfg::THREADS, Cfg::MINBLOCKS)
scatter_pass_kernel(const PassParams<BinFn, NextFn> P) {
  using S = PassSmem<Cfg, FROM_SEQ>;
  constexpr int TILE = Cfg::TILE, THREADS = Cfg::THREADS, NB = Cfg::NB, BPT = Cfg::BPT;
  static_assert(TILE <= 65536, "tile-local positions are 16 bit");
  static_assert(!PEER || NB >= MAX_PEERS, "one bin per owner");
  extern __shared__ __align__(16) unsigned char smem_raw[];
  S &sm = *reinterpret_cast<S *>(smem_raw);
  const unsigned tid = threadIdx.x, lane = tid & 31u, warp = tid >> 5;

  const long long t_start = clock64();
  if (tid == 0) sm.tile = atomicAdd(P.ticket, 1u);
  {
    uint4 *zw = reinterpret_cast<uint4 *>(sm.whist[warp]);
#pragma unroll
    for (int j = 0; j < NB / 4; j += 32) if (j + (int)lane < NB / 4) zw[j + lane] = make_uint4(0, 0, 0, 0);
    if constexpr (Cfg::RANK == 0) {
      uint4 *zm = reinterpret_cast<uint4 *>(sm.match + warp * NB);
#pragma unroll
      for (int j = 0; j < NB / 4; j += 32) if (j + (int)lane < NB / 4) zm[j + lane] = make_uint4(0, 0, 0, 0);
    }
  }
  if constexpr (HAS_NEXT)
    for (int b = tid; b < NB; b += THREADS) sm.next[b] = 0;
  if constexpr (PEER) {
    static_assert(sizeof(PeerTable) % 8 == 0, "copied as 64-bit words");
    if (tid < sizeof(PeerTable) / 8) reinterpret_cast<uint64_t *>(&sm.peer)[tid] = reinterpret_cast<const uint64_t *>(P.peer)[tid];
  }
  uint32_t gbase[BPT];
#pragma unroll
  for (int q = 0; q < BPT; ++q) gbase[q] = (NB >= THREADS || tid < NB) ? __ldg(P.gbase + tid * BPT + q) : 0;
  static_assert(!(SEGS && FROM_SEQ), "only a record source can be segmented");
  uint32_t nsegs = 0;
  if constexpr (SEGS) {
    nsegs = P.segs->nsegs;
    for (uint32_t i = tid; i <= nsegs; i += THREADS) sm.seg_tp[i] = P.segs->tile_prefix[i];
  }
  if constexpr (FROM_SEQ) { if (tid == 0) sm.skip_write = 0; }
  int64_t n_in = FROM_SEQ ? P.sv.nstarts : (SEGS ? 0 : (int64_t)*P.n_records);
  __syncthreads();
  const uint32_t tile = sm.tile;
  int64_t q0 = (int64_t)tile * TILE;
  if constexpr (SEGS) {
    {
      if (tile >= sm.seg_tp[nsegs]) return;
      uint32_t lo = 0, hi = nsegs;
      while (hi - lo > 1) {
        const uint32_t mid = (lo + hi) >> 1;
        if (sm.seg_tp[mid] <= tile) lo = mid; else hi = mid;
      }
      const int64_t base = (int64_t)lo * (int64_t)P.segs->stride;
      q0 = base + (int64_t)(tile - sm.seg_tp[lo]) * TILE;
      n_in = base + (int64_t)P.segs->count[lo];
    }
  }
  if (q0 >= n_in) return;
  if (P.trace && tid == 0) P.trace[(size_t)tile * 8] = (unsigned long long)t_start;

  bool special = false;
  if constexpr (FROM_SEQ) special = tile_pack<TILE, THREADS>(P.sv, q0, sm.tc);
  const bool touches_end = FROM_SEQ && (P.sv.s0 + q0 + TILE + P.sv.k > P.sv.L);
  if (q0 + TILE <= n_in && !special && !touches_end)
    pass_tile<Cfg, FROM_SEQ, true, BinFn, NextFn, HAS_NEXT, PEER>(P, sm, tile, q0, n_in, gbase, special);
  else
    pass_tile<Cfg, FROM_SEQ, false, BinFn, NextFn, HAS_NEXT, PEER>(P, sm, tile, q0, n_in, gbase, special);

  if constexpr (HAS_NEXT) {
    __syncthreads();
    for (int b = tid; b < NB; b += THREADS) {
      const uint32_t c = sm.next[b];
      if (c) atomicAdd(P.hist_next + b, c);
    }
  }
}

template <int NB>
__global__ void __launch_bounds__(NB)
scan_hist_kernel(const uint32_t *__restrict__ hist, uint32_t *__restrict__ gbase, uint64_t *n) {
  __shared__ uint32_t part[NB / 32];
  const unsigned tid = threadIdx.x, lane = tid & 31u, warp = tid >> 5;
  const uint32_t v = hist[tid];
  const uint32_t incl = warp_incl_scan(v);
  if (lane == 31) part[warp] = incl;
  __syncthreads();
  uint32_t add = 0;
  uint64_t tot = 0;
#pragma unroll
  for (int j = 0; j < NB / 32; ++j) {
    if (j < (int)warp) add += part[j];
    tot += part[j];
  }
  gbase[tid] = incl - v + add;
  if (n && tid == 0) *n = tot;
}

struct PeerPtrs { uint64_t *keys[MAX_PEERS]; uint32_t *pos[MAX_PEERS]; };
__global__ void __launch_bounds__(RADIX)
owner_offsets_kernel(const uint64_t *__restrict__ matrix, int nparts, int rank, uint64_t cap, PeerPtrs ptrs,
                     uint32_t *gbase, PeerTable *tab, uint64_t *info) {
  const int b = threadIdx.x;
  if (b == 0) {
    info[1] = 0;
    uint64_t run = 0;
    for (int o = 0; o < RADIX; ++o) { gbase[o] = (uint32_t)run; if (o < nparts) run += matrix[(size_t)rank * nparts + o]; }
  }
  __syncthreads();
  if (b < MAX_PEERS) {
    uint64_t before = 0, total = 0;
    if (b < nparts)
      for (int src = 0; src < nparts; ++src) {
        const uint64_t c = matrix[(size_t)src * nparts + b];
        if (src < rank) before += c;
        total += c;
      }
    tab->keys[b] = b < nparts ? ptrs.keys[b] : nullptr;
    tab->pos[b] = b < nparts ? ptrs.pos[b] : nullptr;
    tab->delta[b] = (int64_t)before - (int64_t)gbase[b];
    tab->counts[b] = nullptr;
    if (b == rank) info[0] = total;
    if (total > cap) info[1] = 1;
  }
  if (b == 0) { tab->cap = cap; tab->rank = (uint32_t)rank; tab->region = 0; }
}

template <int THREADS, int ITEMS>
__global__ void __launch_bounds__(THREADS)
hist_all_kernel(const SeqView sv, uint32_t *common , uint32_t *ind , const int stride) {
  constexpr int TILE = THREADS * ITEMS;
  __shared__ TileCodes<TILE> tc;
  __shared__ uint32_t sh_common[RADIX];
  __shared__ uint32_t sh_ind[MAX_PASSES][RADIX];
  const unsigned tid = threadIdx.x, lane = tid & 31u, warp = tid >> 5;
  const int k = sv.k, R = num_passes(k);
  for (int b = tid; b < RADIX; b += THREADS) sh_common[b] = 0;
  for (int b = tid; b < R * RADIX; b += THREADS) (&sh_ind[0][0])[b] = 0;
  const int64_t tiles = ceil_div<int64_t>(sv.nstarts, TILE);
  for (int64_t tile = blockIdx.x; tile < tiles; tile += gridDim.x) {
    const int64_t q0 = tile * TILE;
    __syncthreads();
    const bool special = tile_pack<TILE, THREADS>(sv, q0, tc);
    const int t0 = warp * (32 * ITEMS) + lane;
    if (!special && q0 + TILE <= sv.nstarts) {
#pragma unroll
      for (int i = 0; i < ITEMS; ++i) atomicAdd(&sh_common[tile_c4<TILE>(tc, t0 + i * 32)], 1u);
      for (int e = tid; e < R * 32; e += THREADS) {
        const int r = e >> 5, t = e & 31, lo = k - 4 * r - 4;
        if (t < lo) {
          atomicSub(&sh_ind[r][tile_c4<TILE>(tc, t)], 1u);
          atomicAdd(&sh_ind[r][tile_c4<TILE>(tc, TILE + t)], 1u);
        }
      }
    } else {
#pragma unroll
      for (int i = 0; i < ITEMS; ++i) {
        const int t = t0 + i * 32;
        if (tile_valid<TILE>(sv, tc, q0, t, special)) {
          const uint64_t key = tile_key<TILE>(tc, t, k);
          for (int r = 0; r < R; ++r) atomicAdd(&sh_ind[r][(uint32_t)(key >> (r * RADIX_BITS)) & (RADIX - 1)], 1u);
        }
      }
    }
  }
  __syncthreads();
  for (int b = tid; b < RADIX; b += THREADS) {
    const uint32_t c = sh_common[b];
    if (c) atomicAdd(common + b, c);
  }
  for (int b = tid; b < R * RADIX; b += THREADS) {
    const uint32_t c = (&sh_ind[0][0])[b];
    if (c) atomicAdd(ind + (size_t)(b / RADIX) * stride + (b % RADIX), c);
  }
}

__global__ void __launch_bounds__(RADIX)
hist_finish_kernel(int k, const uint32_t *__restrict__ common, uint32_t *hist ,
                   uint32_t *gbase , const int stride, uint64_t *n) {
  __shared__ uint32_t part[RADIX / 32];
  const unsigned tid = threadIdx.x, lane = tid & 31u, warp = tid >> 5;
  const int r = blockIdx.x;
  const int m = min(4, k - 4 * r);
  const int s = 2 * (4 - m);
  uint32_t v = hist[(size_t)r * stride + tid];
  if (tid < (1u << (2 * m))) {
    for (uint32_t c = tid << s; c < ((tid + 1u) << s); ++c) v += common[c];
  }
  hist[(size_t)r * stride + tid] = v;
  const uint32_t incl = warp_incl_scan(v);
  if (lane == 31) part[warp] = incl;
  __syncthreads();
  uint32_t add = 0;
  uint64_t tot = 0;
#pragma unroll
  for (int j = 0; j < RADIX / 32; ++j) {
    if (j < (int)warp) add += part[j];
    tot += part[j];
  }
  gbase[(size_t)r * stride + tid] = incl - v + add;
  if (r == 0 && tid == 0) *n = tot;
}

template <int THREADS, int ITEMS, class BinFn>
__global__ void __launch_bounds__(THREADS)
hist_seq_kernel(const SeqView sv, uint32_t *hist, BinFn bin) {
  constexpr int TILE = THREADS * ITEMS;
  __shared__ TileCodes<TILE> tc;
  __shared__ uint32_t sh[MAX_NB];
  const unsigned tid = threadIdx.x;
  for (int b = tid; b < MAX_NB; b += THREADS) sh[b] = 0;
  const int64_t tiles = ceil_div<int64_t>(sv.nstarts, TILE);
  for (int64_t tile = blockIdx.x; tile < tiles; tile += gridDim.x) {
    const int64_t q0 = tile * TILE;
    __syncthreads();
    const bool special = tile_pack<TILE, THREADS>(sv, q0, tc);
    const int t0 = tid * ITEMS;
    const uint64_t kmask = key_mask(sv.k);
    uint64_t key = tile_key<TILE>(tc, t0, sv.k);
    static_assert(ITEMS <= 17, "incoming bases fit two 16-base words");
    const int p0 = t0 + sv.k;
    const uint64_t inc = ((uint64_t(tc.codes[p0 >> 4]) << 32) | tc.codes[(p0 >> 4) + 1]) << (2 * (p0 & 15));
    if (!special && q0 + TILE <= sv.nstarts && sv.s0 + q0 + TILE + sv.k <= sv.L) {
#pragma unroll
      for (int i = 0; i < ITEMS; ++i) {
        if (i > 0) key = ((key << 2) | ((inc >> (64 - 2 * i)) & 3u)) & kmask;
        atomicAdd(&sh[bin(key)], 1u);
      }
    } else {
#pragma unroll
      for (int i = 0; i < ITEMS; ++i) {
        if (i > 0) key = ((key << 2) | ((inc >> (64 - 2 * i)) & 3u)) & kmask;
        if (tile_valid<TILE>(sv, tc, q0, t0 + i, special)) atomicAdd(&sh[bin(key)], 1u);
      }
    }
  }
  __syncthreads();
  for (int b = tid; b < MAX_NB; b += THREADS) {
    uint32_t c = sh[b];
    if (c) atomicAdd(hist + b, c);
  }
}

template <int THREADS, class BinFn>
__global__ void __launch_bounds__(THREADS)
hist_rec_kernel(const uint64_t *keys, int64_t n_host, const uint64_t *n_dev, uint32_t *hist, BinFn bin) {
  __shared__ uint32_t sh[MAX_NB];
  const int64_t n = n_dev ? (int64_t)*n_dev : n_host;
  for (int b = threadIdx.x; b < MAX_NB; b += THREADS) sh[b] = 0;
  __syncthreads();
  for (int64_t i = (int64_t)blockIdx.x * THREADS + threadIdx.x; i < n; i += (int64_t)gridDim.x * THREADS)
    atomicAdd(&sh[bin(ld_stream_u64(keys + i))], 1u);
  __syncthreads();
  for (int b = threadIdx.x; b < MAX_NB; b += THREADS) {
    uint32_t c = sh[b];
    if (c) atomicAdd(hist + b, c);
  }
}

template <int THREADS, class BinFn>
__global__ void __launch_bounds__(THREADS)
hist_seg_kernel(const uint64_t *keys, const TileSegs *seg, uint32_t *hist, BinFn bin) {
  __shared__ uint32_t sh[MAX_NB];
  for (int b = threadIdx.x; b < MAX_NB; b += THREADS) sh[b] = 0;
  __syncthreads();
  const uint32_t nsegs = seg->nsegs;
  for (uint32_t r = 0; r < nsegs; ++r) {
    const int64_t n = (int64_t)seg->count[r];
    const uint64_t *src = keys + (uint64_t)r * seg->stride;
    for (int64_t i = (int64_t)blockIdx.x * THREADS + threadIdx.x; i < n; i += (int64_t)gridDim.x * THREADS)
      atomicAdd(&sh[bin(ld_stream_u64(src + i))], 1u);
  }
  __syncthreads();
  for (int b = threadIdx.x; b < MAX_NB; b += THREADS) {
    uint32_t c = sh[b];
    if (c) atomicAdd(hist + b, c);
  }
}

__global__ void __launch_bounds__(MAX_SEGS)
tile_segs_kernel(const uint64_t *__restrict__ counts, int nsegs, uint64_t stride, uint32_t tile, TileSegs *seg, uint64_t *n) {
  __shared__ uint32_t part_t[MAX_SEGS / 32];
  __shared__ uint64_t part_c[MAX_SEGS / 32];
  __shared__ uint32_t over;
  const unsigned tid = threadIdx.x, lane = tid & 31u, warp = tid >> 5;
  if (tid == 0) over = 0;
  __syncthreads();
  uint64_t c = (int)tid < nsegs ? counts[tid] : 0;
  if (c > stride) over = 1;
  __syncthreads();
  if (over) c = 0;
  const uint32_t t = (uint32_t)((c + tile - 1) / tile);
  const uint32_t it = warp_incl_scan(t);
  const uint64_t ic = warp_incl_scan64(c);
  if (lane == 31) { part_t[warp] = it; part_c[warp] = ic; }
  __syncthreads();
  uint32_t bt = 0, tt = 0;
  uint64_t tc = 0;
  for (int w = 0; w < MAX_SEGS / 32; ++w) { if (w < (int)warp) bt += part_t[w]; tt += part_t[w]; tc += part_c[w]; }
  seg->tile_prefix[tid] = bt + it - t;
  seg->count[tid] = (uint32_t)c;
  if (tid == 0) {
    seg->tile_prefix[MAX_SEGS] = tt;
    seg->stride = stride; seg->total = tc; seg->nsegs = (uint32_t)nsegs; seg->tile = tile; seg->overflow = over; seg->pad = 0;
    *n = tc;
  }
  if ((int)tid == nsegs) seg->tile_prefix[nsegs] = tt;
}
__global__ void seg_compact_kernel(const uint64_t *__restrict__ keys, const uint32_t *__restrict__ pay, const TileSegs *seg,
                                   uint64_t *__restrict__ okeys, uint32_t *__restrict__ opay) {
  const uint32_t nsegs = seg->nsegs;
  uint64_t dst = 0;
  for (uint32_t r = 0; r < nsegs; ++r) {
    const int64_t n = (int64_t)seg->count[r];
    const uint64_t src = (uint64_t)r * seg->stride;
    for (int64_t i = (int64_t)blockIdx.x * blockDim.x + threadIdx.x; i < n; i += (int64_t)gridDim.x * blockDim.x) {
      okeys[dst + i] = ld_stream_u64(keys + src + i);
      opay[dst + i] = ld_stream_u32(pay + src + i);
    }
    dst += (uint64_t)n;
  }
}
__global__ void region_sample_kernel(const SeqView sv, int stride, uint32_t mask, uint32_t *hist ) {
  __shared__ uint32_t sh[MAX_NB];
  for (int b = threadIdx.x; b < MAX_NB; b += blockDim.x) sh[b] = 0;
  __syncthreads();
  const int64_t nsamp = sv.nstarts / stride;
  const uint64_t kmask = key_mask(sv.k);
  for (int64_t i = (int64_t)blockIdx.x * blockDim.x + threadIdx.x; i < nsamp; i += (int64_t)gridDim.x * blockDim.x) {
    const uint8_t *p = sv.base + i * stride;
    uint64_t w = 0;
    bool clean = true;
    for (int j = 0; j < sv.k; ++j) { const uint8_t c = p[j]; clean &= (c | 0x20) != 'n'; w = (w << 2) | ((c >> 1) & 3u); }
    if (clean) atomicAdd(&sh[(uint32_t)mix64(w & kmask) & mask], 1u);
  }
  __syncthreads();
  for (int b = threadIdx.x; b < MAX_NB; b += blockDim.x) {
    const uint32_t c = sh[b];
    if (c) atomicAdd(hist + b, c);
  }
}
__global__ void region_estimate_kernel(const uint32_t *hist, int nb, int stride, uint32_t *est) {
  __shared__ uint32_t m;
  if (threadIdx.x == 0) m = 0;
  __syncthreads();
  uint32_t mine = 0;
  for (int b = threadIdx.x; b < nb; b += blockDim.x) mine = max(mine, hist[b]);
  atomicMax(&m, mine);
  __syncthreads();
  if (threadIdx.x == 0) est[0] = m * (uint32_t)stride;
}
__global__ void region_gbase_kernel(uint32_t *gbase, int nb, uint32_t cap, uint32_t *overflow) {
  for (int b = threadIdx.x; b < MAX_NB; b += blockDim.x) gbase[b] = b < nb ? (uint32_t)b * cap : 0;
  if (threadIdx.x == 0) *overflow = 0;
}

}
```

Before: 25.63 billion.

## Add MSD radix path: two scatter passes then per-bucket local CTA sorts

For 8-bit, four-pass grouped builds with regions, the LSD multi-pass sort is replaced by an MSD scheme. The first pass from the sequence bins by the top digit into regions, and a second segmented pass scatters into 65536 sampled sub-buckets with planned capacities. Each sub-bucket is then sorted in shared memory by a local CTA kernel, with separate handling for oversized buckets, which removes the later global scatter passes and the group-fix pass. The costs are extra sampling, capacity planning based on the sample, and new overflow paths.

Result: no change. 25.87 billion, median of 6 (+0.9%).

```diff
diff --git a/kmer_hasher_b200/csrc/api.cu b/kmer_hasher_b200/csrc/api.cu
--- a/kmer_hasher_b200/csrc/api.cu
+++ b/kmer_hasher_b200/csrc/api.cu
@@ -17,6 +17,7 @@
 #include "common.cuh"
 #include "csr.cuh"
 #include "lookback.cuh"
+#include "msd.cuh"
 #include "probe.cuh"
 #include "sort.cuh"
 #include "windows.cuh"
@@ -493,6 +494,12 @@
 static int g_scatter_bitmap = 0;
 static int g_hash_cas = 0;
 static int g_fix_cap = 0;
+static int g_msd = -1;
+static std::atomic<uint64_t> g_msd_oversized{0};
+static int msd_mode() {
+  if (g_msd < 0) { const char *e = getenv("KMG_MSD"); g_msd = e ? atoi(e) : 1; }
+  return g_msd;
+}
 static SortPlan grouped_plan(int64_t n_upper) {
   if (g_hash_bits > 0) {
     const int rb = g_hash_rb > 0 && g_hash_bits % g_hash_rb == 0 ? g_hash_rb : (g_hash_bits % 8 == 0 ? 8 : 9);
@@ -528,6 +535,11 @@
   if (key && !strcmp(key, "scatter_bitmap")) { g_scatter_bitmap = value != 0; return KMG_OK; }
   if (key && !strcmp(key, "scatter_shape")) { g_scatter_shape = value; return KMG_OK; }
   if (key && !strcmp(key, "no_regions")) { g_no_regions = value; return KMG_OK; }
+  if (key && !strcmp(key, "msd")) {
+    if (value < 0 || value > 2) return fail(KMG_ERR_ARG, "msd must be 0 (LSD), 1 (MSD where it applies) or 2 (tests: sub-regions without slack)");
+    g_msd = value;
+    return KMG_OK;
+  }
   if (key && !strcmp(key, "hash_bits")) {
     if (value != 0 && (value < 8 || value > 56 || (value % 8 && value % 9 && value % 10))) return fail(KMG_ERR_ARG, "hash_bits must be 0 (auto) or a multiple of 8, 9 or 10 in [8,56]");
     g_hash_bits = value;
@@ -554,6 +566,8 @@
   if (key && !strcmp(key, "rank_variant")) return ctx_init() == KMG_OK ? rank_variant() : -1;
   if (key && !strcmp(key, "unstable_rebuilds")) return (int64_t)g_unstable_rebuilds.load();
   if (key && !strcmp(key, "region_rebuilds")) return (int64_t)g_region_rebuilds.load();
+  if (key && !strcmp(key, "msd_oversized")) return (int64_t)g_msd_oversized.load();
+  if (key && !strcmp(key, "msd")) return msd_mode();
   if (key && !strcmp(key, "hash_bits")) return grouped_plan(arg).bits();
   if (key && !strcmp(key, "hash_rb")) return grouped_plan(arg).rb;
   return -1;
@@ -578,13 +592,18 @@
 constexpr int REGION_SAMPLE_STRIDE = 251;
 constexpr int SORT_TILE_MIN = 4096;
 
-template <class Cfg, bool FROM_SEQ, class BinFn, class NextFn, bool HAS_NEXT, bool PEER = false, bool SEGS = false>
+template <class Cfg, bool FROM_SEQ, class BinFn, class NextFn, bool HAS_NEXT, bool PEER = false, bool SEGS = false, bool MSD = false>
 static int launch_pass_cfg(const char *name, const PassParams<BinFn, NextFn> &P, int64_t n_upper, cudaStream_t s, int extra_tiles = 0) {
   using S = PassSmem<Cfg, FROM_SEQ>;
   if constexpr (!FROM_SEQ && !PEER && !SEGS) {
-    if (P.segs) return launch_pass_cfg<Cfg, FROM_SEQ, BinFn, NextFn, HAS_NEXT, PEER, true>(name, P, n_upper, s, extra_tiles);
-  }
-  auto kern = scatter_pass_kernel<Cfg, FROM_SEQ, BinFn, NextFn, HAS_NEXT, PEER, SEGS>;
+    if (P.segs) {
+      if constexpr (!HAS_NEXT) {
+        if (P.msd) return launch_pass_cfg<Cfg, FROM_SEQ, BinFn, NextFn, HAS_NEXT, PEER, true, true>(name, P, n_upper, s, extra_tiles);
+      }
+      return launch_pass_cfg<Cfg, FROM_SEQ, BinFn, NextFn, HAS_NEXT, PEER, true>(name, P, n_upper, s, extra_tiles);
+    }
+  }
+  auto kern = scatter_pass_kernel<Cfg, FROM_SEQ, BinFn, NextFn, HAS_NEXT, PEER, SEGS, MSD>;
   CU(cudaFuncSetAttribute(kern, cudaFuncAttributeMaxDynamicSharedMemorySize, (int)sizeof(S)));
   const int64_t tiles = ceil_div<int64_t>(n_upper, Cfg::TILE) + extra_tiles;
   if (tiles == 0) return KMG_OK;
@@ -750,27 +769,44 @@
   uint32_t *pr = nullptr, *d_over = nullptr;
   TileSegs *segs = nullptr;
   uint32_t h_over = 0;
+  const bool msd_plan = msd_mode() != 0 && rb == 8 && R == 4;
+  bool msd = false;
+  uint32_t msd_slots = 0, h_nbig = 0, small_cap = 0;
+  uint32_t *d_sub = nullptr, *d_off = nullptr, *ps = nullptr;
+  uint64_t *ks = nullptr, *d_sc = nullptr;
   regions = regions && R > 1 && NB <= MAX_SEGS && n_upper <= (int64_t)1600000000;
   const uint32_t cap = (uint32_t)(((uint64_t)(n_upper / NB) * 5 / 4 + 4096 + 15) & ~uint64_t(15));
   if (regions && g_no_regions == 2) {
   } else if (regions && n_upper >= (int64_t)REGION_SAMPLE_STRIDE * 4096) {
-    uint32_t *d_s = nullptr, h_est = 0;
-    TRY(dalloc(&d_s, (size_t)MAX_NB + 1, s));
+    uint32_t *d_s = nullptr, h_info[2] = {0, 0};
+    const size_t words = msd_plan ? (size_t)MSD_SUB + 2 : (size_t)MAX_NB + 1;
+    TRY(dalloc(&d_s, words, s));
     int rc0 = KMG_OK;
-    if (cudaMemsetAsync(d_s, 0, (MAX_NB + 1) * sizeof(uint32_t), s) != cudaSuccess) rc0 = fail(KMG_ERR_CUDA, "memset failed");
+    if (msd_plan) rc0 = dalloc(&d_sub, (size_t)MSD_SUB + 1, s);
+    if (rc0 == KMG_OK && cudaMemsetAsync(d_s, 0, words * sizeof(uint32_t), s) != cudaSuccess) rc0 = fail(KMG_ERR_CUDA, "memset failed");
     if (rc0 == KMG_OK) {
       const unsigned g = (unsigned)std::min<int64_t>(ceil_div<int64_t>(n_upper / REGION_SAMPLE_STRIDE, 256), (int64_t)g_ctx.sms * 8);
-      region_sample_kernel<<<g, 256, 0, s>>>(sv, REGION_SAMPLE_STRIDE, mask, d_s);
-      region_estimate_kernel<<<1, 256, 0, s>>>(d_s, NB, REGION_SAMPLE_STRIDE, d_s + MAX_NB);
-      if (cudaMemcpyAsync(&h_est, d_s + MAX_NB, 4, cudaMemcpyDeviceToHost, s) != cudaSuccess || cudaStreamSynchronize(s) != cudaSuccess)
+      if (msd_plan) {
+        region_sample_kernel<<<g, 256, 0, s>>>(sv, REGION_SAMPLE_STRIDE, 16, MSD_SUB - 1, d_s);
+        msd_plan_kernel<<<1, 1024, 0, s>>>(d_s, n_upper, REGION_SAMPLE_STRIDE, msd_mode() == 2 ? 0 : 1, d_sub, d_s + MSD_SUB);
+      } else {
+        region_sample_kernel<<<g, 256, 0, s>>>(sv, REGION_SAMPLE_STRIDE, 0, mask, d_s);
+        region_estimate_kernel<<<1, 256, 0, s>>>(d_s, NB, REGION_SAMPLE_STRIDE, d_s + MAX_NB);
+      }
+      if (cudaMemcpyAsync(h_info, d_s + words - (msd_plan ? 2 : 1), (msd_plan ? 2 : 1) * sizeof(uint32_t), cudaMemcpyDeviceToHost, s) != cudaSuccess ||
+          cudaStreamSynchronize(s) != cudaSuccess)
         rc0 = fail(KMG_ERR_CUDA, "region estimate failed: %s", cudaGetErrorString(cudaGetLastError()));
     }
     dfree(d_s, s);
-    TRY(rc0);
-    if ((uint64_t)h_est * 10 > (uint64_t)cap * 9) regions = false;
+    if (rc0 != KMG_OK) { dfree(d_sub, s); return rc0; }
+    if ((uint64_t)h_info[0] * 10 > (uint64_t)cap * 9) regions = false;
+    else if (msd_plan && h_info[1] != 0xFFFFFFFFu) { msd = true; msd_slots = h_info[1]; }
+    if (!msd) dfree(d_sub, s);
   } else if (regions) {
     regions = false;
   }
+  uint32_t h_cnt[4] = {0, 0, 0, 0};
+  uint32_t *fixmem = nullptr;
   auto body = [&]() -> int {
     PassParams<DigitBin, DigitBin> P{};
     P.sv = sv; P.keys_out = ka; P.pos_out = pa;
@@ -779,7 +815,52 @@
     P.hashed = 1;
     P.dbg = g_sort_dbg;
     P.bin = DigitBin{0, mask}; P.next = DigitBin{rb, mask};
-    if (regions) {
+    if (msd) {
+      TRY(dalloc(&kr, (size_t)NB * cap, s));
+      TRY(dalloc(&pr, (size_t)NB * cap, s));
+      TRY(dalloc(&ks, (size_t)msd_slots, s));
+      TRY(dalloc(&ps, (size_t)msd_slots, s));
+      TRY(dalloc(&d_counts, (size_t)MAX_SEGS, s));
+      TRY(dalloc(&d_sc, (size_t)MSD_SUB, s));
+      TRY(dalloc(&d_off, (size_t)2 * MSD_SUB + 2, s));
+      TRY(dalloc(&d_over, 4, s));
+      TRY(dalloc(&segs, 1, s));
+      uint32_t *n_big = d_off + MSD_SUB + 1, *big_list = n_big + 1;
+      CU(cudaMemsetAsync(d_counts, 0, MAX_SEGS * sizeof(uint64_t), s));
+      CU(cudaMemsetAsync(d_sc, 0, MSD_SUB * sizeof(uint64_t), s));
+      CU(cudaMemsetAsync(n_big, 0, sizeof(uint32_t), s));
+      LAUNCH("region_gbase", s, region_gbase_kernel<<<1, 256, 0, s>>>(sc.gbase(0), NB, cap, d_over));
+      P.keys_out = kr; P.pos_out = pr;
+      P.bin = DigitBin{24, mask};
+      P.bin_counts = d_counts; P.bin_cap = cap; P.bin_overflow = d_over;
+      TRY((launch_pass<true, DigitBin, DigitBin, false>("sort_pass_seq", P, n_upper, s, rb)));
+      LAUNCH("tile_segs", s, tile_segs_kernel<<<1, MAX_SEGS, 0, s>>>(d_counts, NB, (uint64_t)cap, record_tile(rb), segs, &sc.stats()->n));
+      PassParams<DigitBin, DigitBin> P1{};
+      P1.keys_in = kr; P1.pos_in = pr; P1.keys_out = ks; P1.pos_out = ps;
+      P1.gbase = d_sub; P1.status = sc.status; P1.ticket = sc.ticket(1); P1.epoch = 2;
+      P1.n_records = &sc.stats()->n;
+      P1.segs = segs; P1.msd = 1;
+      P1.bin_counts = d_sc; P1.bin_overflow = d_over;
+      P1.dbg = g_sort_dbg;
+      P1.bin = DigitBin{16, mask}; P1.next = DigitBin{16, mask};
+      TRY((launch_pass<false, DigitBin, DigitBin, false>("sort_pass_msd", P1, n_upper, s, rb, NB)));
+      LAUNCH("msd_scan", s, msd_scan_kernel<<<1, 1024, 0, s>>>(d_sc, d_sub, d_off, sc.stats(), d_over));
+      FixLists fl{};
+      small_cap = g_fix_cap > 0 ? (uint32_t)g_fix_cap : (uint32_t)std::max<int64_t>(1 << 20, n_upper / 8);
+      fl.big_cap = 1 << 16;
+      TRY(dalloc(&fixmem, 4 + 2 * (size_t)fl.big_cap, s));
+      CU(cudaMemsetAsync(fixmem, 0, 4 * sizeof(uint32_t), s));
+      fl.counters = fixmem;
+      fl.big_tasks = reinterpret_cast<uint2 *>(fixmem + 4);
+      CU(cudaFuncSetAttribute(msd_local_kernel, cudaFuncAttributeMaxDynamicSharedMemorySize, (int)sizeof(LocalSmem)));
+      LAUNCH("msd_local", s, msd_local_kernel<<<g_ctx.sms * 2, LS_THREADS, sizeof(LocalSmem), s>>>(ks, ps, d_sub, d_off, big_list, n_big, ka, pa, fl, rank_variant() >= 3));
+      uint32_t *wa = reinterpret_cast<uint32_t *>(kb);
+      LAUNCH("msd_oversized", s, msd_oversized_kernel<<<g_ctx.sms, LS_THREADS, 0, s>>>(ks, ps, d_sub, d_off, big_list, n_big, wa, wa + n_upper, ka, pa, fl, rank_variant() >= 3));
+      LAUNCH("big_fix", s, big_fix_kernel<1024><<<g_ctx.sms, 1024, 0, s>>>(ka, pa, kb, pb, fl));
+      CU(cudaMemcpyAsync(h_cnt, fl.counters, 4 * sizeof(uint32_t), cudaMemcpyDeviceToHost, s));
+      CU(cudaMemcpyAsync(&h_nbig, n_big, sizeof(uint32_t), cudaMemcpyDeviceToHost, s));
+      CU(cudaMemcpyAsync(&h_over, d_over, 4, cudaMemcpyDeviceToHost, s));
+    } else if (regions) {
       TRY(dalloc(&kr, (size_t)NB * cap, s));
       TRY(dalloc(&pr, (size_t)NB * cap, s));
       TRY(dalloc(&d_counts, (size_t)MAX_SEGS, s));
@@ -812,19 +893,24 @@
     return KMG_OK;
   };
   int rc = body();
-  uint32_t h_cnt[4] = {0, 0, 0, 0};
-  uint32_t *fixmem = nullptr;
-  if (rc == KMG_OK) rc = fix_groups(sc, plan.bits(), ka, pa, kb, pb, n_upper, s, h_cnt, &fixmem);
+  if (rc == KMG_OK && !msd) rc = fix_groups(sc, plan.bits(), ka, pa, kb, pb, n_upper, s, h_cnt, &fixmem);
   if (rc == KMG_OK) rc = finish_index(ix, sc, ka, pa, n_upper, s, true);
   dfree(fixmem, s);
   dfree(kr, s); dfree(pr, s); dfree(d_counts, s); dfree(d_over, s); dfree(segs, s);
-  *overflow = h_cnt[2] != 0;
+  dfree(ks, s); dfree(ps, s); dfree(d_sc, s); dfree(d_off, s); dfree(d_sub, s);
+  *overflow = h_cnt[2] != 0 || (msd && h_cnt[0] > small_cap);
   *region_overflow = h_over != 0;
+  if (rc == KMG_OK && h_nbig) g_msd_oversized.fetch_add(h_nbig);
   if (log_on()) fprintf(stderr, "[kmergpu] grouped build on %d bits: %u short and %u long groups fixed\n", plan.bits(), h_cnt[0], h_cnt[1]);
   ix->hbits = plan.bits();
   const double N = (double)ix->N, L = (double)sv.avail;
   if (!regions) prof_bytes("hist_seq", L);
   prof_bytes("sort_pass_seq", L + 12 * N);
+  if (msd) {
+    prof_bytes("sort_pass_msd", 24 * N);
+    prof_bytes("msd_local", 24 * N);
+    return rc;
+  }
   if (R > 2) prof_bytes("sort_pass_hist", 24 * N * (R - 2));
   if (R > 1) prof_bytes("sort_pass", 24 * N);
   prof_bytes("group_detect", 8 * N);
diff --git a/kmer_hasher_b200/csrc/msd.cuh b/kmer_hasher_b200/csrc/msd.cuh
--- /dev/null
+++ b/kmer_hasher_b200/csrc/msd.cuh
@@ -0,0 +1,374 @@
+#pragma once
+#include "common.cuh"
+#include "csr.cuh"
+#include "sort.cuh"
+
+namespace kmg {
+
+constexpr int MSD_SUB = 1 << 16;
+constexpr int LS_THREADS = 256, LS_ITEMS = 24;
+constexpr int LS_CAP = LS_THREADS * LS_ITEMS;
+constexpr int REPAIR_CHUNK = LS_CAP - 8;
+static_assert((REPAIR_CHUNK + 3) / 3 <= (LS_THREADS / 32) * RADIX, "the repair's task list fits the bin counters");
+constexpr int LOCAL_MAX = REPAIR_CHUNK;
+static_assert(LS_THREADS == RADIX, "one bin per thread in the scan");
+
+__global__ void __launch_bounds__(1024)
+msd_plan_kernel(const uint32_t *__restrict__ sample, int64_t n_upper, int stride, int slack, uint32_t *__restrict__ sub_base,
+                uint32_t *info) {
+  constexpr int PER = MSD_SUB / 1024;
+  __shared__ uint64_t part[32];
+  __shared__ uint32_t top;
+  const unsigned tid = threadIdx.x, lane = tid & 31u, warp = tid >> 5;
+  if (tid == 0) top = 0;
+  const uint64_t mean = (uint64_t)ceil_div<int64_t>(n_upper, MSD_SUB);
+  auto cap = [&](uint32_t c) -> uint64_t {
+    const uint64_t est = (uint64_t)c * (uint64_t)stride;
+    const uint64_t v = slack ? 2 * mean + 2 * (est > mean ? est - mean : 0) : mean;
+    return (v + 16 + 15) & ~uint64_t(15);
+  };
+  uint64_t mine = 0;
+  uint32_t sampled = 0;
+  for (int j = 0; j < PER; ++j) {
+    const uint32_t c = sample[tid * PER + j];
+    sampled += c;
+    mine += cap(c);
+  }
+  sampled += __shfl_xor_sync(FULL, sampled, 1);
+  sampled += __shfl_xor_sync(FULL, sampled, 2);
+  const uint64_t incl = warp_incl_scan64(mine);
+  if (lane == 31) part[warp] = incl;
+  __syncthreads();
+  if ((tid & 3) == 0) atomicMax(&top, sampled);
+  uint64_t run = incl - mine, total = 0;
+  for (int w = 0; w < 32; ++w) { if (w < (int)warp) run += part[w]; total += part[w]; }
+  for (int j = 0; j < PER; ++j) { sub_base[tid * PER + j] = (uint32_t)run; run += cap(sample[tid * PER + j]); }
+  __syncthreads();
+  if (tid == 0) {
+    sub_base[MSD_SUB] = (uint32_t)total;
+    info[0] = top * (uint32_t)stride;
+    info[1] = total > (uint64_t)INT32_MAX ? 0xFFFFFFFFu : (uint32_t)total;
+  }
+}
+
+__global__ void __launch_bounds__(1024)
+msd_scan_kernel(const uint64_t *__restrict__ counts, const uint32_t *__restrict__ sub_base, uint32_t *__restrict__ off,
+                IndexStats *st, uint32_t *overflow) {
+  constexpr int PER = MSD_SUB / 1024;
+  __shared__ uint64_t part[32];
+  __shared__ uint32_t over;
+  const unsigned tid = threadIdx.x, lane = tid & 31u, warp = tid >> 5;
+  if (tid == 0) over = 0;
+  __syncthreads();
+  uint64_t mine = 0;
+  bool bad = false;
+#pragma unroll 16
+  for (int j = 0; j < PER; ++j) {
+    const int i = tid * PER + j;
+    const uint64_t c = counts[i];
+    bad |= c > (uint64_t)(sub_base[i + 1] - sub_base[i]);
+    mine += c;
+  }
+  if (bad) over = 1;
+  __syncthreads();
+  if (over) mine = 0;
+  const uint64_t incl = warp_incl_scan64(mine);
+  if (lane == 31) part[warp] = incl;
+  __syncthreads();
+  uint64_t run = incl - mine, total = 0;
+  for (int w = 0; w < 32; ++w) { if (w < (int)warp) run += part[w]; total += part[w]; }
+#pragma unroll 16
+  for (int j = 0; j < PER; ++j) { off[tid * PER + j] = (uint32_t)run; if (!over) run += counts[tid * PER + j]; }
+  if (tid == 0) {
+    off[MSD_SUB] = (uint32_t)total;
+    st->n = total;
+    if (over) *overflow = 1;
+  }
+}
+
+__device__ __forceinline__ uint32_t cta_excl_scan256(uint32_t v, uint32_t *part , uint32_t *tot) {
+  const unsigned lane = threadIdx.x & 31u, warp = threadIdx.x >> 5;
+  const uint32_t incl = warp_incl_scan(v);
+  if (lane == 31) part[warp] = incl;
+  __syncthreads();
+  uint32_t before = 0, all = 0;
+#pragma unroll
+  for (int w = 0; w < LS_THREADS / 32; ++w) { if (w < (int)warp) before += part[w]; all += part[w]; }
+  *tot = all;
+  __syncthreads();
+  return incl - v + before;
+}
+
+template <bool SINGLE, int IT>
+__device__ __forceinline__ void cta_digit_pass(const uint32_t *src, uint32_t *dst, const uint64_t *keys, uint32_t n, int shift,
+                                               uint32_t (*whist)[RADIX], uint32_t *bins, uint32_t *part, const bool lane_ordered) {
+  constexpr int WARPS = LS_THREADS / 32;
+  const unsigned tid = threadIdx.x, lane = tid & 31u, warp = tid >> 5;
+  const unsigned lt = lanemask_lt();
+  static_assert(IT <= LS_ITEMS, "a tile fits the shared-memory arrays");
+  for (uint32_t t0 = 0; t0 < n; t0 += LS_THREADS * IT) {
+    for (int b = lane; b < RADIX; b += 32) whist[warp][b] = 0;
+    __syncwarp();
+    uint32_t idx[IT], rk[IT];
+    const uint32_t wb = t0 + warp * (32 * IT) + lane;
+#pragma unroll
+    for (int i = 0; i < IT; ++i) {
+      const uint32_t j = wb + i * 32;
+      idx[i] = j < n ? (src ? src[j] : j) : 0;
+    }
+    if (lane_ordered) {
+      const bool wfull = wb - lane + 32 * IT <= n;
+#pragma unroll
+      for (int i = 0; i < IT; ++i) {
+        const bool ok = wb + i * 32 < n;
+        const uint32_t d = (uint32_t)(keys[idx[i]] >> shift) & (RADIX - 1);
+        rk[i] = 0xFFFFFFFFu;
+        if (ok) rk[i] = (d << 16) | atomicAdd(&whist[warp][d], 1u);
+        if (!wfull) __syncwarp();
+      }
+    } else
+#pragma unroll
+    for (int i = 0; i < IT; ++i) {
+      const bool ok = wb + i * 32 < n;
+      const uint32_t d = ok ? (uint32_t)(keys[idx[i]] >> shift) & (RADIX - 1) : RADIX + lane;
+      const unsigned peers = __match_any_sync(FULL, d);
+      const int leader = __ffs(peers) - 1;
+      uint32_t r0 = 0;
+      if (ok && (int)lane == leader) { r0 = whist[warp][d]; whist[warp][d] = r0 + __popc(peers); }
+      r0 = __shfl_sync(FULL, r0, leader);
+      rk[i] = ok ? (d << 16) | (r0 + __popc(peers & lt)) : 0xFFFFFFFFu;
+      __syncwarp();
+    }
+    __syncthreads();
+    {
+      const unsigned b = tid;
+      uint32_t c[WARPS], tot = 0;
+#pragma unroll
+      for (int w = 0; w < WARPS; ++w) { c[w] = whist[w][b]; tot += c[w]; }
+      uint32_t start;
+      if constexpr (SINGLE) { uint32_t all; start = cta_excl_scan256(tot, part, &all); }
+      else { start = bins[b]; bins[b] = start + tot; }
+#pragma unroll
+      for (int w = 0; w < WARPS; ++w) { whist[w][b] = start; start += c[w]; }
+    }
+    __syncthreads();
+#pragma unroll
+    for (int i = 0; i < IT; ++i)
+      if (rk[i] != 0xFFFFFFFFu) dst[whist[warp][rk[i] >> 16] + (rk[i] & 0xFFFFu)] = idx[i];
+    __syncthreads();
+  }
+}
+
+__device__ __forceinline__ void cta_digit_bases(const uint32_t *src, const uint64_t *keys, uint32_t n, int shift, uint32_t *bins,
+                                                uint32_t *part) {
+  bins[threadIdx.x] = 0;
+  __syncthreads();
+  for (uint32_t j = threadIdx.x; j < n; j += LS_THREADS)
+    atomicAdd(&bins[(uint32_t)(keys[src ? src[j] : j] >> shift) & (RADIX - 1)], 1u);
+  __syncthreads();
+  const uint32_t v = bins[threadIdx.x];
+  uint32_t all;
+  const uint32_t e = cta_excl_scan256(v, part, &all);
+  bins[threadIdx.x] = e;
+  __syncthreads();
+}
+
+__device__ __forceinline__ void file_boundary(const uint32_t *w, const uint64_t *keys, uint32_t n, uint32_t out0, uint32_t j,
+                                              uint64_t y, uint32_t *tasks, uint32_t *ntask, const FixLists &fl) {
+  const uint32_t lo = (uint32_t)y;
+  uint32_t s = j - 1;
+  while (s > 0) {
+    const uint64_t v = keys[w[s - 1]];
+    if ((uint32_t)v != lo) break;
+    if (v != y) return;
+    --s;
+  }
+  uint32_t e = j + 1;
+  while (e < n && (uint32_t)keys[w[e]] == lo) ++e;
+  if (e - s > (uint32_t)SMALL_GROUP) {
+    const uint32_t t = atomicAdd(fl.counters + 1, 1u);
+    if (t < fl.big_cap) fl.big_tasks[t] = make_uint2(out0 + s, out0 + e); else fl.counters[2] = 1;
+    return;
+  }
+  bool split = false;
+  for (uint32_t a = s + 1; a < e && !split; ++a) {
+    const uint64_t v = keys[w[a]];
+    if (v != keys[w[a - 1]])
+      for (uint32_t m = s; m + 1 < a; ++m)
+        if (keys[w[m]] == v) { split = true; break; }
+  }
+  if (split) tasks[atomicAdd(ntask, 1u)] = s;
+}
+__device__ __forceinline__ uint32_t sort_group(uint32_t *w, const uint64_t *keys, uint32_t n, uint32_t s) {
+  const uint32_t lo = (uint32_t)keys[w[s]];
+  uint32_t e = s + 1;
+  while (e < n && (uint32_t)keys[w[e]] == lo) ++e;
+  for (uint32_t a = s + 1; a < e; ++a) {
+    const uint32_t ia = w[a];
+    const uint64_t v = keys[ia];
+    uint32_t m = a;
+    while (m > s && keys[w[m - 1]] > v) { w[m] = w[m - 1]; --m; }
+    w[m] = ia;
+  }
+  return e;
+}
+
+__device__ __forceinline__ void cta_repair(uint32_t *w, const uint64_t *keys, uint32_t n, uint32_t out0, uint32_t *tasks,
+                                           uint32_t *ntask, uint32_t *dirty, const FixLists &fl) {
+  const unsigned tid = threadIdx.x;
+  for (uint32_t c0 = 0; c0 < n; c0 += REPAIR_CHUNK) {
+    if (tid == 0) *ntask = 0;
+    __syncthreads();
+    for (uint32_t j = c0 + tid; j < min(n, c0 + REPAIR_CHUNK); j += LS_THREADS) {
+      if (j == 0) continue;
+      const uint64_t x = keys[w[j]], y = keys[w[j - 1]];
+      if ((uint32_t)x != (uint32_t)y || x == y) continue;
+      file_boundary(w, keys, n, out0, j, y, tasks, ntask, fl);
+    }
+    __syncthreads();
+    const uint32_t nt = *ntask;
+    if (tid == 0) *dirty += nt;
+    for (uint32_t t = tid; t < nt; t += LS_THREADS) sort_group(w, keys, n, tasks[t]);
+    __syncthreads();
+  }
+}
+
+struct LocalSmem {
+  uint64_t keys[LS_CAP];
+  uint32_t pos[LS_CAP];
+  uint32_t w[LS_CAP];
+  uint32_t whist[LS_THREADS / 32][RADIX];
+  uint32_t part[LS_THREADS / 32];
+  uint32_t ntask, dirty;
+  uint32_t next[3];
+  alignas(8) uint64_t bar[2];
+};
+
+__device__ __forceinline__ void bulk_arm(uint64_t *bar, void *dst, const void *src, uint32_t bytes) {
+  asm volatile("mbarrier.arrive.expect_tx.shared::cta.b64 _, [%0], %1;" ::"r"(smem_addr(bar)), "r"(bytes) : "memory");
+  asm volatile("cp.async.bulk.shared::cluster.global.mbarrier::complete_tx::bytes [%0], [%1], %2, [%3];"
+               ::"r"(smem_addr(dst)), "l"(src), "r"(bytes), "r"(smem_addr(bar)) : "memory");
+}
+__device__ __forceinline__ void bulk_wait(uint64_t *bar, uint32_t parity) {
+  asm volatile(
+      "{\n\t.reg .pred p;\n\t"
+      "KMG_LWAIT:\n\t"
+      "mbarrier.try_wait.parity.shared::cta.b64 p, [%0], %1;\n\t"
+      "@p bra KMG_LDONE;\n\t"
+      "bra KMG_LWAIT;\n\t"
+      "KMG_LDONE:\n\t}" ::"r"(smem_addr(bar)), "r"(parity) : "memory");
+}
+__device__ __forceinline__ void prefetch_l2(const void *src, uint32_t bytes) {
+  asm volatile("cp.async.bulk.prefetch.L2.global [%0], %1;" ::"l"(src), "r"(bytes) : "memory");
+}
+
+template <int IT>
+__device__ __forceinline__ void local_sort(LocalSmem &sm, uint32_t n, uint32_t o, uint32_t parity, uint64_t *__restrict__ kout,
+                                           uint32_t *__restrict__ pout, const FixLists &fl, const bool lane_ordered) {
+  bulk_wait(&sm.bar[0], parity);
+  cta_digit_pass<true, IT>(nullptr, sm.w, sm.keys, n, 0, sm.whist, nullptr, sm.part, lane_ordered);
+  cta_digit_pass<true, IT>(sm.w, sm.w, sm.keys, n, 8, sm.whist, nullptr, sm.part, lane_ordered);
+  bulk_wait(&sm.bar[1], parity);
+  uint32_t *tasks = &sm.whist[0][0];
+  const unsigned lane = threadIdx.x & 31u;
+  for (uint32_t j0 = 0; j0 < n; j0 += LS_THREADS) {
+    const uint32_t j = j0 + threadIdx.x;
+    const bool ok = j < n;
+    const uint32_t i = ok ? sm.w[j] : 0;
+    const uint64_t x = sm.keys[i];
+    if (ok) { kout[o + j] = x; pout[o + j] = sm.pos[i]; }
+    uint64_t y = __shfl_up_sync(FULL, x, 1);
+    if (lane == 0 && j > 0 && ok) y = sm.keys[sm.w[j - 1]];
+    if (ok && j > 0 && (uint32_t)x == (uint32_t)y && x != y) file_boundary(sm.w, sm.keys, n, o, j, y, tasks, &sm.ntask, fl);
+  }
+  __syncthreads();
+  const uint32_t nt = sm.ntask;
+  for (uint32_t t = threadIdx.x; t < nt; t += LS_THREADS) {
+    const uint32_t s = tasks[t], e = sort_group(sm.w, sm.keys, n, s);
+    for (uint32_t a = s; a < e; ++a) { const uint32_t i = sm.w[a]; kout[o + a] = sm.keys[i]; pout[o + a] = sm.pos[i]; }
+  }
+  if (threadIdx.x == 0) sm.dirty = nt;
+}
+
+__global__ void __launch_bounds__(LS_THREADS, 2)
+msd_local_kernel(const uint64_t *__restrict__ kin, const uint32_t *__restrict__ pin, const uint32_t *__restrict__ sub_base,
+                 const uint32_t *__restrict__ off, uint32_t *big_list, uint32_t *n_big, uint64_t *__restrict__ kout,
+                 uint32_t *__restrict__ pout, FixLists fl, const bool lane_ordered) {
+  extern __shared__ __align__(16) unsigned char smem_raw[];
+  LocalSmem &sm = *reinterpret_cast<LocalSmem *>(smem_raw);
+  const unsigned tid = threadIdx.x;
+  if (tid == 0) {
+    asm volatile("mbarrier.init.shared::cta.b64 [%0], 1;" ::"r"(smem_addr(&sm.bar[0])) : "memory");
+    asm volatile("mbarrier.init.shared::cta.b64 [%0], 1;" ::"r"(smem_addr(&sm.bar[1])) : "memory");
+    asm volatile("fence.proxy.async.shared::cta;" ::: "memory");
+    const uint32_t b = blockIdx.x;
+    sm.next[0] = off[b]; sm.next[1] = off[b + 1] - sm.next[0]; sm.next[2] = sub_base[b];
+  }
+  __syncthreads();
+  uint32_t parity = 0;
+  for (uint32_t b = blockIdx.x; b < (uint32_t)MSD_SUB; b += gridDim.x) {
+    const uint32_t o = sm.next[0], n = sm.next[1], base = sm.next[2];
+    __syncthreads();
+    if (tid == 0) {
+      if (n > 0 && n <= (uint32_t)LOCAL_MAX) {
+        const uint32_t m = (n + 3) & ~3u;
+        bulk_arm(&sm.bar[0], sm.keys, kin + base, m * 8);
+        bulk_arm(&sm.bar[1], sm.pos, pin + base, m * 4);
+      } else if (n > 0) {
+        big_list[atomicAdd(n_big, 1u)] = b;
+      }
+      sm.ntask = 0;
+      const uint32_t nb = b + gridDim.x;
+      if (nb < (uint32_t)MSD_SUB) {
+        const uint32_t no = off[nb], nn = off[nb + 1] - no, nbase = sub_base[nb];
+        sm.next[0] = no; sm.next[1] = nn; sm.next[2] = nbase;
+        if (nn > 0 && nn <= (uint32_t)LOCAL_MAX) {
+          const uint32_t m = (nn + 3) & ~3u;
+          prefetch_l2(kin + nbase, m * 8);
+          prefetch_l2(pin + nbase, m * 4);
+        }
+      }
+    }
+    __syncthreads();
+    if (n == 0 || n > (uint32_t)LOCAL_MAX) continue;
+    if (n <= LS_THREADS * 8) local_sort<8>(sm, n, o, parity, kout, pout, fl, lane_ordered);
+    else if (n <= LS_THREADS * 16) local_sort<16>(sm, n, o, parity, kout, pout, fl, lane_ordered);
+    else local_sort<LS_ITEMS>(sm, n, o, parity, kout, pout, fl, lane_ordered);
+    parity ^= 1u;
+    __syncthreads();
+    if (tid == 0 && sm.dirty) atomicAdd(fl.counters + 0, sm.dirty);
+  }
+}
+
+__global__ void __launch_bounds__(LS_THREADS)
+msd_oversized_kernel(const uint64_t *__restrict__ kin, const uint32_t *__restrict__ pin, const uint32_t *__restrict__ sub_base,
+                     const uint32_t *__restrict__ off, const uint32_t *big_list, const uint32_t *n_big, uint32_t *wa, uint32_t *wb,
+                     uint64_t *__restrict__ kout, uint32_t *__restrict__ pout, FixLists fl, const bool lane_ordered) {
+  __shared__ uint32_t whist[LS_THREADS / 32][RADIX];
+  __shared__ uint32_t bins[RADIX];
+  __shared__ uint32_t part[LS_THREADS / 32];
+  __shared__ uint32_t ntask, dirty;
+  const unsigned tid = threadIdx.x;
+  const uint32_t count = *n_big;
+  for (uint32_t t = blockIdx.x; t < count; t += gridDim.x) {
+    const uint32_t b = big_list[t];
+    const uint32_t o = off[b], n = off[b + 1] - o;
+    const uint64_t *keys = kin + sub_base[b];
+    const uint32_t *pos = pin + sub_base[b];
+    if (tid == 0) dirty = 0;
+    cta_digit_bases(nullptr, keys, n, 0, bins, part);
+    cta_digit_pass<false, LS_ITEMS>(nullptr, wa + o, keys, n, 0, whist, bins, part, lane_ordered);
+    cta_digit_bases(wa + o, keys, n, 8, bins, part);
+    cta_digit_pass<false, LS_ITEMS>(wa + o, wb + o, keys, n, 8, whist, bins, part, lane_ordered);
+    cta_repair(wb + o, keys, n, o, &whist[0][0], &ntask, &dirty, fl);
+    for (uint32_t j = tid; j < n; j += LS_THREADS) {
+      const uint32_t i = wb[o + j];
+      kout[o + j] = keys[i];
+      pout[o + j] = pos[i];
+    }
+    __syncthreads();
+    if (tid == 0 && dirty) atomicAdd(fl.counters + 0, dirty);
+  }
+}
+
+}
diff --git a/kmer_hasher_b200/csrc/sort.cuh b/kmer_hasher_b200/csrc/sort.cuh
--- a/kmer_hasher_b200/csrc/sort.cuh
+++ b/kmer_hasher_b200/csrc/sort.cuh
@@ -79,6 +79,7 @@
   uint32_t pos_add;
   const PeerTable *peer;
   const TileSegs *segs;
+  uint32_t msd;
   uint64_t *bin_counts;
   uint32_t bin_cap;
   uint32_t *bin_overflow;
@@ -220,16 +221,18 @@
       "KMG_DONE:\n\t}" ::"r"(b) : "memory");
 }
 
-template <class Cfg, bool FROM_SEQ, bool FULL, class BinFn, class NextFn, bool HAS_NEXT, bool PEER>
+template <class Cfg, bool FROM_SEQ, bool FULL, class BinFn, class NextFn, bool HAS_NEXT, bool PEER, bool MSD>
 __device__ __forceinline__ void pass_tile(const PassParams<BinFn, NextFn> &P, PassSmem<Cfg, FROM_SEQ> &sm,
                                           const uint32_t tile, const int64_t q0, const int64_t n_in,
-                                          const uint32_t (&gbase)[Cfg::BPT], const bool special) {
+                                          const uint32_t (&gbase)[Cfg::BPT], const uint32_t (&bcap)[Cfg::BPT],
+                                          const uint32_t tfirst, const uint32_t cbase, const bool special) {
   using S = PassSmem<Cfg, FROM_SEQ>;
   constexpr int TILE = Cfg::TILE, THREADS = Cfg::THREADS, ITEMS = Cfg::ITEMS, WARPS = S::WARPS, NB = Cfg::NB, BPT = Cfg::BPT;
   const unsigned tid = threadIdx.x, lane = tid & 31u, warp = tid >> 5;
   const int t0 = warp * (32 * ITEMS) + lane;
   const bool owns = NB >= THREADS || tid < NB;
   const int b0 = tid * BPT;
+  constexpr bool REGIONS = (FROM_SEQ || MSD) && !PEER;
 #define KMG_STAMP(slot) do { if (P.trace && tid == 0) P.trace[(size_t)tile * 8 + (slot)] = clock64(); } while (0)
   KMG_STAMP(1);
 
@@ -335,7 +338,7 @@
       }
       uint64_t sw[BPT];
 #pragma unroll
-      for (int q = 0; q < BPT; ++q) { sw[q] = st_pack(tile == 0 ? ST_INCL : ST_AGG, P.epoch, cnt[q]); mine += cnt[q]; }
+      for (int q = 0; q < BPT; ++q) { sw[q] = st_pack(tile == tfirst ? ST_INCL : ST_AGG, P.epoch, cnt[q]); mine += cnt[q]; }
       st_status<BPT>(P.status + (size_t)tile * NB + b0, sw);
     }
     const uint32_t incl = warp_incl_scan(mine);
@@ -399,7 +402,7 @@
     bool done[BPT];
 #pragma unroll
     for (int q = 0; q < BPT; ++q) { excl[q] = 0; done[q] = false; }
-    if (tile > 0 && !(P.dbg & 1u)) {
+    if (tile > tfirst && !(P.dbg & 1u)) {
       constexpr int LB = Cfg::LB;
       int64_t t = (int64_t)tile - 1;
       bool all_done = false;
@@ -407,7 +410,7 @@
         uint64_t w[LB][BPT];
 #pragma unroll
         for (int j = 0; j < LB; ++j) {
-          if (t - j >= 0) ld_status<BPT>(P.status + (size_t)(t - j) * NB + b0, w[j]);
+          if (t - j >= (int64_t)tfirst) ld_status<BPT>(P.status + (size_t)(t - j) * NB + b0, w[j]);
           else {
 #pragma unroll
             for (int q = 0; q < BPT; ++q) w[j][q] = st_pack(ST_INCL, P.epoch, 0);
@@ -445,10 +448,10 @@
     for (int q = 0; q < BPT; ++q) {
       const int64_t go = (int64_t)gbase[q] + (int64_t)excl[q] - (int64_t)lstart[q];
       sm.goff[b0 + q] = (int32_t)go;
-      if constexpr (FROM_SEQ && !PEER) {
+      if constexpr (REGIONS) {
         if (P.bin_counts) {
-          if (excl[q] + cnt[q] > P.bin_cap) { *P.bin_overflow = 1; sm.skip_write = 1; }
-          if (q0 + TILE >= n_in) P.bin_counts[b0 + q] = excl[q] + cnt[q];
+          if (excl[q] + cnt[q] > bcap[q]) { *P.bin_overflow = 1; sm.skip_write = 1; }
+          if (q0 + TILE >= n_in) P.bin_counts[cbase + b0 + q] = excl[q] + cnt[q];
         }
       }
       if constexpr (PEER) {
@@ -462,7 +465,7 @@
   KMG_STAMP(6);
 
   bool drop = false;
-  if constexpr (FROM_SEQ && !PEER) drop = sm.skip_write != 0;
+  if constexpr (REGIONS) drop = sm.skip_write != 0;
   bool aligned_out = false;
   if constexpr (PEER) aligned_out = !(P.dbg & 4u);
   if (aligned_out) {
@@ -507,7 +510,7 @@
         dst += sm.peer.delta[b];
         room = (uint64_t)(sm.peer.region ? local : dst) < sm.peer.cap;
       }
-      if constexpr (FROM_SEQ && !PEER) room = !drop;
+      if constexpr (REGIONS) room = !drop;
       if (room && !(P.dbg & 2u)) {
         kout[dst] = kk;
         if constexpr (FROM_SEQ) pout[dst] = (uint32_t)(P.sv.s0 + q0 + 1) + P.pos_add + sm.pos[s];
@@ -520,7 +523,7 @@
 #undef KMG_STAMP
 }
 
-template <class Cfg, bool FROM_SEQ, class BinFn, class NextFn, bool HAS_NEXT, bool PEER = false, bool SEGS = false>
+template <class Cfg, bool FROM_SEQ, class BinFn, class NextFn, bool HAS_NEXT, bool PEER = false, bool SEGS = false, bool MSD = false>
 __global__ void __launch_bounds__(Cfg::THREADS, Cfg::MINBLOCKS)
 scatter_pass_kernel(const PassParams<BinFn, NextFn> P) {
   using S = PassSmem<Cfg, FROM_SEQ>;
@@ -549,20 +552,25 @@
     static_assert(sizeof(PeerTable) % 8 == 0, "copied as 64-bit words");
     if (tid < sizeof(PeerTable) / 8) reinterpret_cast<uint64_t *>(&sm.peer)[tid] = reinterpret_cast<const uint64_t *>(P.peer)[tid];
   }
-  uint32_t gbase[BPT];
-#pragma unroll
-  for (int q = 0; q < BPT; ++q) gbase[q] = (NB >= THREADS || tid < NB) ? __ldg(P.gbase + tid * BPT + q) : 0;
   static_assert(!(SEGS && FROM_SEQ), "only a record source can be segmented");
+  static_assert(!MSD || (SEGS && !HAS_NEXT && !PEER), "an MSD pass reads the first pass's regions and needs no next histogram");
+  uint32_t gbase[BPT], bcap[BPT];
+#pragma unroll
+  for (int q = 0; q < BPT; ++q) {
+    gbase[q] = (!MSD && (NB >= THREADS || tid < NB)) ? __ldg(P.gbase + tid * BPT + q) : 0;
+    bcap[q] = P.bin_cap;
+  }
   uint32_t nsegs = 0;
   if constexpr (SEGS) {
     nsegs = P.segs->nsegs;
     for (uint32_t i = tid; i <= nsegs; i += THREADS) sm.seg_tp[i] = P.segs->tile_prefix[i];
   }
-  if constexpr (FROM_SEQ) { if (tid == 0) sm.skip_write = 0; }
+  if constexpr (FROM_SEQ || MSD) { if (tid == 0) sm.skip_write = 0; }
   int64_t n_in = FROM_SEQ ? P.sv.nstarts : (SEGS ? 0 : (int64_t)*P.n_records);
   __syncthreads();
   const uint32_t tile = sm.tile;
   int64_t q0 = (int64_t)tile * TILE;
+  uint32_t tfirst = 0, cbase = 0;
   if constexpr (SEGS) {
     {
       if (tile >= sm.seg_tp[nsegs]) return;
@@ -574,6 +582,18 @@
       const int64_t base = (int64_t)lo * (int64_t)P.segs->stride;
       q0 = base + (int64_t)(tile - sm.seg_tp[lo]) * TILE;
       n_in = base + (int64_t)P.segs->count[lo];
+      if constexpr (MSD) {
+        tfirst = sm.seg_tp[lo];
+        cbase = lo * NB;
+        if (NB >= THREADS || tid < NB) {
+#pragma unroll
+          for (int q = 0; q < BPT; ++q) {
+            const uint32_t *g = P.gbase + cbase + tid * BPT + q;
+            gbase[q] = __ldg(g);
+            bcap[q] = __ldg(g + 1) - gbase[q];
+          }
+        }
+      }
     }
   }
   if (q0 >= n_in) return;
@@ -583,9 +603,9 @@
   if constexpr (FROM_SEQ) special = tile_pack<TILE, THREADS>(P.sv, q0, sm.tc);
   const bool touches_end = FROM_SEQ && (P.sv.s0 + q0 + TILE + P.sv.k > P.sv.L);
   if (q0 + TILE <= n_in && !special && !touches_end)
-    pass_tile<Cfg, FROM_SEQ, true, BinFn, NextFn, HAS_NEXT, PEER>(P, sm, tile, q0, n_in, gbase, special);
+    pass_tile<Cfg, FROM_SEQ, true, BinFn, NextFn, HAS_NEXT, PEER, MSD>(P, sm, tile, q0, n_in, gbase, bcap, tfirst, cbase, special);
   else
-    pass_tile<Cfg, FROM_SEQ, false, BinFn, NextFn, HAS_NEXT, PEER>(P, sm, tile, q0, n_in, gbase, special);
+    pass_tile<Cfg, FROM_SEQ, false, BinFn, NextFn, HAS_NEXT, PEER, MSD>(P, sm, tile, q0, n_in, gbase, bcap, tfirst, cbase, special);
 
   if constexpr (HAS_NEXT) {
     __syncthreads();
@@ -840,7 +860,7 @@
     dst += (uint64_t)n;
   }
 }
-__global__ void region_sample_kernel(const SeqView sv, int stride, uint32_t mask, uint32_t *hist ) {
+__global__ void region_sample_kernel(const SeqView sv, int stride, int shift, uint32_t mask, uint32_t *hist ) {
   __shared__ uint32_t sh[MAX_NB];
   for (int b = threadIdx.x; b < MAX_NB; b += blockDim.x) sh[b] = 0;
   __syncthreads();
@@ -851,7 +871,10 @@
     uint64_t w = 0;
     bool clean = true;
     for (int j = 0; j < sv.k; ++j) { const uint8_t c = p[j]; clean &= (c | 0x20) != 'n'; w = (w << 2) | ((c >> 1) & 3u); }
-    if (clean) atomicAdd(&sh[(uint32_t)mix64(w & kmask) & mask], 1u);
+    if (clean) {
+      const uint32_t b = (uint32_t)(mix64(w & kmask) >> shift) & mask;
+      if (mask < MAX_NB) atomicAdd(&sh[b], 1u); else atomicAdd(hist + b, 1u);
+    }
   }
   __syncthreads();
   for (int b = threadIdx.x; b < MAX_NB; b += blockDim.x) {
```
